# flkraus/bayesian-yolov3

Hardware: AMD Instinct MI355X
Metric: img/s at T=30 MC-dropout, 608x608 (higher is better)
Workload: dtype f32 via split-f16 (hi+lo fp16 pairs, 3 fp16 MFMA products, fp32 accumulate)

## Files before the change

### bayesian-yolov3_amd/byolo/_lib.py

```python
import ctypes
import os

_HERE = os.path.dirname(os.path.abspath(__file__))
LIB_PATH = os.environ.get("BYOLO_LIB") or os.path.join(_HERE, "libbyolo.so")

OK, ERR_ARG, ERR_STATE, ERR_HIP, ERR_NOMEM, ERR_RANGE = 0, -1, -2, -3, -4, -5
DET_STANDARD, DET_ALEATORIC, DET_EPISTEMIC = 0, 1, 2
NMS_AGNOSTIC, NMS_TWO_CLASS, NMS_PER_CLASS = 0, 1, 2
NMS_MAX_CLASSES = 128
NORM_BN, NORM_DROPOUT = 1, 2
AUG_SATURATION, AUG_BRIGHTNESS, AUG_HUE = 1, 2, 3
AUG_COLORED_SALT_N_PEPPER, AUG_SALT_N_PEPPER, AUG_GAUSSIAN = 1, 2, 3


class ByoloError(RuntimeError):
    def __init__(self, code, msg):
        super().__init__("libbyolo error %d: %s" % (code, msg))
        self.code = code


class Cfg(ctypes.Structure):
    _fields_ = [("img_h", ctypes.c_int32), ("img_w", ctypes.c_int32), ("img_c", ctypes.c_int32),
                ("cls_cnt", ctypes.c_int32), ("drop_prob", ctypes.c_float), ("max_out", ctypes.c_int32),
                ("iou_thresh", ctypes.c_float), ("nms_mode", ctypes.c_int32), ("keep_all_outputs", ctypes.c_int32)]


class PlanOpts(ctypes.Structure):
    _fields_ = [(n, ctypes.c_int32) for n in (
        "struct_bytes", "graphs", "serialize_convs", "serialize_heads", "dedup", "lowmain", "kx3", "p1", "b2b", "kx3_wide", "wino_split", "wino_split_min_c",
        "wino_split_bn", "wino_split_rounds", "winograd", "wino_fused", "stream1x1", "gemm_stream", "ksplit", "streamk",
        "plain_epilogue", "wshift_per_layer", "nms_general", "wino_split_persist", "wino_split_feed")] + [(n, ctypes.c_float) for n in (
        "wino_split_min_gflop", "wino_split_chunk_mb", "wino_min_gflop", "wino_chunk_mb", "wino_min_ratio")]


class AugPlan(ctypes.Structure):
    _fields_ = [(n, ctypes.c_int32) for n in ("y0", "x0", "ch", "cw", "row0", "rescale", "flip", "blur_k", "color_op", "noise_op")] + \
               [("color_param", ctypes.c_float), ("noise_param", ctypes.c_float), ("noise_key", ctypes.c_uint64)]


EVAL_MAX_GT, EVAL_MAX_UNC, EVAL_RECORD_HEAD = 1024, 16, 7


class EvalCfg(ctypes.Structure):
    _fields_ = [(n, ctypes.c_int32) for n in ("struct_bytes", "row_len", "obj_idx", "cls_start_idx", "cls_cnt", "n_unc")] + \
               [("unc_cols", ctypes.c_int32 * EVAL_MAX_UNC), ("iou_thresh", ctypes.c_float), ("min_score", ctypes.c_float)]


EVAL_LOC_WORDS, EVAL_LOC_MAX_LAYERS, EVAL_LOC_MAX_PRIORS = 6, 8, 16


class EvalLocCfg(ctypes.Structure):
    _fields_ = [(n, ctypes.c_int32) for n in ("struct_bytes", "layer_col", "prior_col", "n_layers")] + \
               [(n, ctypes.c_int32 * EVAL_LOC_MAX_LAYERS) for n in ("lh", "lw", "n_priors")] + \
               [(n, (ctypes.c_float * EVAL_LOC_MAX_PRIORS) * EVAL_LOC_MAX_LAYERS) for n in ("prior_w", "prior_h")]


EVAL_LADDER_MAX = 16


class EvalLadderCfg(ctypes.Structure):
    _fields_ = [("struct_bytes", ctypes.c_int32), ("n_thr", ctypes.c_int32), ("thresholds", ctypes.c_float * EVAL_LADDER_MAX)]


EVAL_SUBSETS_MAX = 16


class EvalSubsetsCfg(ctypes.Structure):
    _fields_ = [("struct_bytes", ctypes.c_int32), ("n_subsets", ctypes.c_int32), ("lo", ctypes.c_float * EVAL_SUBSETS_MAX),
                ("hi", ctypes.c_float * EVAL_SUBSETS_MAX), ("img_h", ctypes.c_float), ("ignore_thresh", ctypes.c_float),
                ("height_slack", ctypes.c_float), ("ignore_other_classes", ctypes.c_int32)]


class EvalSummary(ctypes.Structure):
    _fields_ = [(n, ctypes.c_int32) for n in ("struct_bytes", "overflow", "record_words", "reserved")] + \
               [(n, ctypes.c_int64) for n in ("n_records", "n_seen", "n_images")]


VOTE_NONE, VOTE_ALE, VOTE_EPI, VOTE_TOTAL = 0, 1, 2, 3


class VoteCfg(ctypes.Structure):
    _fields_ = [("struct_bytes", ctypes.c_int32), ("var", ctypes.c_int32)] + \
               [(n, ctypes.c_float) for n in ("sigma_t", "iou_min", "min_score", "var_floor")] + \
               [("ale_col", ctypes.c_int32), ("epi_col", ctypes.c_int32)]
# ... 192 lines not shown
```

### bayesian-yolov3_amd/csrc/byolo_api.hip

```cpp
#include "byolo_internal.h"
#include <cfloat>

static thread_local std::string g_err;

int32_t byolo_fail(byolo_t* h, int32_t code, const char* fmt, ...) {
    char buf[1024];
    va_list ap; va_start(ap, fmt); vsnprintf(buf, sizeof buf, fmt, ap); va_end(ap);
    if (h) h->err = buf; else g_err = buf;
    return code;
}

extern "C" const char* byolo_version(void) { return "byolo 0.7 (gfx950; fp32 MFMA and split-f16 MFMA; abi 7)"; }
extern "C" int32_t byolo_abi_version(void) { return BYOLO_ABI_VERSION; }

extern "C" const char* byolo_last_error(const byolo_t* h) { return h ? h->err.c_str() : g_err.c_str(); }

static void plan_opts_defaults(byolo_plan_opts& o);
static void plan_opts_from_env(byolo_plan_opts& o);

extern "C" int32_t byolo_create(const byolo_cfg* cfg, int32_t device, byolo_t** out) {
    if (!cfg || !out) return fail(nullptr, BYOLO_ERR_ARG, "byolo_create: null argument");
    if (cfg->img_h <= 0 || cfg->img_w <= 0 || cfg->img_c <= 0)
        return fail(nullptr, BYOLO_ERR_ARG, "byolo_create: invalid image size");
    if (cfg->img_h % 32 || cfg->img_w % 32)
        return fail(nullptr, BYOLO_ERR_ARG, "byolo_create: full_img_size must be a multiple of 32 (yolov3.py:207-208)");
    if (cfg->cls_cnt < 1 || cfg->cls_cnt > byk::BYOLO_MAX_CLASSES)
        return fail(nullptr, BYOLO_ERR_ARG, "byolo_create: cls_cnt outside 1 .. 128");
    if (cfg->max_out < 1 || cfg->max_out > 2048) return fail(nullptr, BYOLO_ERR_ARG, "byolo_create: max_out out of [1,2048]");
    if (!(cfg->drop_prob >= 0.f && cfg->drop_prob < 1.f)) return fail(nullptr, BYOLO_ERR_ARG, "byolo_create: drop_prob");
    byolo_t* h = new (std::nothrow) byolo();
    if (!h) return fail(nullptr, BYOLO_ERR_NOMEM, "byolo_create: out of host memory");
    h->cfg = *cfg;
    h->device = device;
    plan_opts_defaults(h->opts);
    plan_opts_from_env(h->opts);
    h->dedup = h->opts.dedup != 0;
    if (const char* e = getenv("BYOLO_PRECISION")) h->precision = (!strcmp(e, "f32") || !strcmp(e, "0")) ? 0 : 1;
    h->prec_requested = h->precision;
    *out = h;
    return BYOLO_OK;
}

static void plan_opts_defaults(byolo_plan_opts& o) {
    memset(&o, 0, sizeof o);
    o.struct_bytes = (int32_t)sizeof o;
    o.graphs = 1; o.serialize_convs = 1; o.serialize_heads = 1; o.dedup = 1; o.lowmain = 1; o.kx3 = 1; o.p1 = 1; o.b2b = 1; o.kx3_wide = 0;
    o.wino_split = 1; o.wino_split_min_c = 256; o.wino_split_bn = 0; o.wino_split_rounds = 0;
    o.winograd = 1; o.wino_fused = 1; o.stream1x1 = 1; o.gemm_stream = 1; o.ksplit = -1; o.streamk = 1; o.plain_epilogue = 1; o.wino_split_persist = 0; o.wino_split_feed = 3;
    o.wino_split_min_gflop = 30.f; o.wino_split_chunk_mb = 1500.f; o.wino_min_gflop = 10.f; o.wino_chunk_mb = 800.f; o.wino_min_ratio = 80.f;
}
static void plan_opts_from_env(byolo_plan_opts& o) {
    auto geti = [](const char* name, int32_t& v) { if (const char* e = getenv(name)) v = atoi(e); };
    auto getf = [](const char* name, float& v) { if (const char* e = getenv(name)) v = (float)atof(e); };
    geti("BYOLO_GRAPHS", o.graphs); geti("BYOLO_SERIALIZE_CONVS", o.serialize_convs); geti("BYOLO_SERIALIZE_HEADS", o.serialize_heads);
    if (const char* e = getenv("BYOLO_NO_DEDUP")) o.dedup = atoi(e) ? 0 : 1;
    geti("BYOLO_LOWMAIN", o.lowmain); geti("BYOLO_KX3", o.kx3); geti("BYOLO_P1", o.p1); geti("BYOLO_B2B", o.b2b); geti("BYOLO_KX3_WIDE", o.kx3_wide);
    geti("BYOLO_WINO_SPLIT", o.wino_split); geti("BYOLO_WINO_SPLIT_MIN_C", o.wino_split_min_c); geti("BYOLO_WINO_SPLIT_BN", o.wino_split_bn);
    geti("BYOLO_WINO_SPLIT_ROUNDS", o.wino_split_rounds); geti("BYOLO_WINOGRAD", o.winograd);
    geti("BYOLO_WINO_FUSED", o.wino_fused); geti("BYOLO_STREAM1X1", o.stream1x1); geti("BYOLO_GEMM_STREAM", o.gemm_stream);
    geti("BYOLO_KSPLIT", o.ksplit); geti("BYOLO_STREAMK", o.streamk); geti("BYOLO_PLAIN_EPILOGUE", o.plain_epilogue); geti("BYOLO_WINO_SPLIT_PERSIST", o.wino_split_persist); geti("BYOLO_WINO_SPLIT_FEED", o.wino_split_feed);
    geti("BYOLO_WSHIFT_PER_LAYER", o.wshift_per_layer); geti("BYOLO_NMS_GENERAL", o.nms_general);
    getf("BYOLO_WINO_SPLIT_MIN_GFLOP", o.wino_split_min_gflop); getf("BYOLO_WINO_SPLIT_CHUNK_MB", o.wino_split_chunk_mb);
    getf("BYOLO_WINO_MIN_GFLOP", o.wino_min_gflop); getf("BYOLO_WINO_CHUNK_MB", o.wino_chunk_mb); getf("BYOLO_WINO_MIN_RATIO", o.wino_min_ratio);
}

static void drop_graphs(byolo_t* h) {
    bool any = false;
    for (auto& g : h->graphs) any = any || g.exec;
    if (any) (void)hipDeviceSynchronize();
    for (auto& g : h->graphs) if (g.exec) (void)hipGraphExecDestroy(g.exec);
    h->graphs.clear();
}

extern "C" int32_t byolo_get_plan_opts(const byolo_t* h, byolo_plan_opts* out) {
    if (!h || !out) return fail(const_cast<byolo_t*>(h), BYOLO_ERR_ARG, "byolo_get_plan_opts: null argument");
    *out = h->opts;
    out->struct_bytes = (int32_t)sizeof *out;
    return BYOLO_OK;
}

extern "C" int32_t byolo_set_plan_opts(byolo_t* h, const byolo_plan_opts* o) {
    if (!h || !o) return fail(h, BYOLO_ERR_ARG, "byolo_set_plan_opts: null argument");
    if (o->struct_bytes != (int32_t)sizeof *o) return fail(h, BYOLO_ERR_ARG, "byolo_set_plan_opts: struct_bytes %d, this library's byolo_plan_opts has %d (include/byolo.h)", o->struct_bytes, (int)sizeof *o);
    if (o->graphs < 0 || o->graphs > 2 || o->serialize_convs < 0 || o->serialize_convs > 2 || o->b2b < 0 || o->b2b > 2 || o->kx3_wide < 0 || o->kx3_wide > 2 ||
        o->wino_split < 0 || o->wino_split > 2 || o->winograd < 0 || o->winograd > 2 || o->wino_fused < 0 || o->wino_fused > 2 || o->stream1x1 < 0 || o->stream1x1 > 2 ||
        o->streamk < 0 || o->streamk > 2 || o->ksplit < -1 || o->ksplit > 64 || (o->wino_split_bn != 0 && o->wino_split_bn != 128 && o->wino_split_bn != 256) ||
        o->wino_split_rounds < 0 || o->wino_split_persist < 0 || o->wino_split_persist > 2 || o->wino_split_feed < 0 || o->wino_split_feed > 3 || !(o->wino_split_chunk_mb > 0.f) || !(o->wino_chunk_mb > 0.f) || !(o->wino_split_min_gflop >= 0.f) || !(o->wino_min_gflop >= 0.f) || !(o->wino_min_ratio >= 0.f))
        return fail(h, BYOLO_ERR_ARG, "byolo_set_plan_opts: a field outside its range (include/byolo.h)");
    const byolo_plan_opts& c = h->opts;
    const bool repack = (o->wshift_per_layer != 0) != (c.wshift_per_layer != 0) || (o->dedup != 0) != (c.dedup != 0) || (o->lowmain != 0) != (c.lowmain != 0) || (o->kx3 != 0) != (c.kx3 != 0) || (o->p1 != 0) != (c.p1 != 0);
    h->opts = *o;
    h->dedup = o->dedup != 0;
    h->plan.B = -1; h->plan.T = -1; ++h->plan_epoch; h->wsm_B = -1;
    if (h->d_blob || !h->graphs.empty()) { HIPCHK(h, hipSetDevice(h->device)); drop_graphs(h); }
    if (repack && h->lowered) { h->lowered = false; h->finalized = false; }
    return BYOLO_OK;
}

extern "C" int32_t byolo_graph_stats(const byolo_t* h, int32_t* n_graphs, int64_t* replays, int64_t* captures, int64_t* updates) {
    if (!h) return BYOLO_ERR_ARG;
    int n = 0; for (const auto& g : h->graphs) n += g.exec != nullptr;
    if (n_graphs) *n_graphs = n;
    if (replays) *replays = h->graph_replays;
    if (captures) *captures = h->graph_captures;
    if (updates) *updates = h->graph_updates;
    return BYOLO_OK;
}

extern "C" int32_t byolo_set_precision(byolo_t* h, int32_t precision) {
    if (!h) return fail(nullptr, BYOLO_ERR_ARG, "byolo_set_precision: null handle");
    if (precision != BYOLO_PREC_F32 && precision != BYOLO_PREC_SPLIT_F16) return fail(h, BYOLO_ERR_ARG, "byolo_set_precision: unknown precision %d", precision);
    h->prec_requested = precision;
    if (precision == BYOLO_PREC_F32) h->prec_note.clear();
    if (precision != h->precision) { h->precision = precision; h->prec_note.clear(); h->finalized = false; h->plan.B = -1; h->plan.T = -1; ++h->plan_epoch; }
    return BYOLO_OK;
}
extern "C" int32_t byolo_get_precision(const byolo_t* h) { return h ? h->precision : BYOLO_ERR_ARG; }

extern "C" int32_t byolo_destroy(byolo_t* h) {
    if (!h) return BYOLO_OK;
    bool on_device = h->d_blob || h->d_ones || h->d_status || !h->graphs.empty() || h->cap_stream;
    for (auto& ps : h->prof) on_device = on_device || ps.ev[0] || !ps.step_ev.empty();
    if (on_device) {
        (void)hipSetDevice(h->device);
        drop_graphs(h);
        if (h->cap_stream) (void)hipStreamDestroy(h->cap_stream);
        if (h->d_blob) (void)hipFree(h->d_blob);
        if (h->d_ones) (void)hipFree(h->d_ones);
        if (h->d_zeros) (void)hipFree(h->d_zeros);
        if (h->ev_convs) (void)hipEventDestroy(h->ev_convs);
        if (h->d_status) (void)hipFree(h->d_status);
        if (h->pc_own) (void)hipFree(h->pc_own);
        if (h->vn_own) (void)hipFree(h->vn_own);
        if (h->vr_tab) (void)hipFree(h->vr_tab);
        if (h->sr_tab) (void)hipFree(h->sr_tab);
        if (h->sr_own) (void)hipFree(h->sr_own);
        if (h->h_status) (void)hipHostFree(h->h_status);
        for (auto& ps : h->prof) {
            for (auto& e : ps.ev) if (e) (void)hipEventDestroy(e);
            for (auto& e : ps.step_ev) (void)hipEventDestroy(e);
// ... 307 lines not shown
                h->aux.push_back({l.H, l.W, l.filters});
                st.raw_tensor = n + (int)h->aux.size() - 1;
                h->last_use.push_back(-1);
            } else if (st.in.n == 2 && any_tile && !all_tile) {
                const int kt = st.in.s[0].tile ? 0 : 1;
                Step part; part.layer = i; part.mode = STEP_PARTIAL;
                part.in.n = 1; part.in.s[0] = st.in.s[kt]; part.in.s[0].tile = false;
                part.c_lo = kt == 0 ? 0 : st.in.s[0].C; part.c_hi = part.c_lo + st.in.s[kt].C;
                h->aux.push_back({l.H, l.W, l.filters});
                part.out_tensor = n + (int)h->aux.size() - 1;
                h->last_use.push_back(-1);
                const int pidx = (int)h->steps.size();
                if (part.in.s[0].layer >= 0) h->last_use[part.in.s[0].layer] = pidx;
                h->steps.push_back(part);
                Step main = st; main.mode = STEP_MAIN; main.addend_tensor = part.out_tensor;
                main.in.n = 1; main.in.s[0] = st.in.s[1 - kt];
                main.c_lo = kt == 0 ? st.in.s[0].C : 0; main.c_hi = main.c_lo + st.in.s[1 - kt].C;
                st = main;
                if (h->opts.lowmain != 0 && l.ksize == 1 && l.stride == 1 && st.in.s[0].sh == 1 && st.in.s[0].layer >= 0 &&
                    !st.in.s[0].tile && (l.H & 1) == 0 && (l.W & 1) == 0 && (l.filters & 3) == 0 && l.fused_residual < 0 && (st.in.s[0].C % 32) == 0) {
                    Step lowst = st; lowst.mode = STEP_PARTIAL; lowst.low = true; lowst.addend_tensor = -1;
                    lowst.in.s[0].sh = 0;
                    h->aux.push_back({l.H / 2, l.W / 2, l.filters, true});
                    lowst.out_tensor = n + (int)h->aux.size() - 1;
                    h->last_use.push_back(-1);
                    const int lidx = (int)h->steps.size();
                    h->last_use[lowst.in.s[0].layer] = lidx;
                    h->steps.push_back(lowst);
                    Step fin; fin.layer = i; fin.mode = STEP_FINISH; fin.out_tensor = l.out_tensor;
                    fin.low_tensor = lowst.out_tensor; fin.addend_tensor = part.out_tensor;
                    fin.c_lo = st.c_lo; fin.c_hi = st.c_hi;
                    const int fidx = (int)h->steps.size();
                    h->last_use[fin.low_tensor] = fidx; h->last_use[fin.addend_tensor] = fidx;
                    h->steps.push_back(fin);
                    continue;
                }
            }
        }
        const int step_idx = (int)h->steps.size();
        for (int k = 0; k < st.in.n; ++k) if (st.in.s[k].layer >= 0) h->last_use[st.in.s[k].layer] = step_idx;
        if (st.addend_tensor >= 0) h->last_use[st.addend_tensor] = step_idx;
        if (l.fused_residual >= 0) h->last_use[h->layers[l.fused_residual].ref[0]] = step_idx;
        h->steps.push_back(st);
    }
    for (auto& st : h->steps) {
        if (!st.is_conv()) continue;
        const Layer& l = h->layers[st.layer];
        const int N = l.filters;
        if (l.direct) { st.tile = -1; st.Npad = N; }
        else { st.tile = conv_pick_tile(N); const int bn = conv_tile_bn(st.tile); st.Npad = (N + bn - 1) / bn * bn; }
        st.wino_ok = !l.direct && l.op == OP_CONV && l.ksize == 3 && l.stride == 1 && st.mode == STEP_NORMAL &&
                     st.in.n == 1 && st.in.s[0].sh == 0 && !st.in.s[0].tile && (l.Cin % 32) == 0 && (N % 4) == 0;
    }
    h->maxC = 1;
    for (const auto& l : h->layers) h->maxC = std::max(h->maxC, l.C);
    decide_loops(h);
    h->lowered = true;
    return BYOLO_OK;
}

int32_t byolo_lower(byolo_t* h) {
    const int n = (int)h->layers.size();
    if (!n) return fail(h, BYOLO_ERR_STATE, "byolo_finalize: empty graph");
    if (!h->n_det) return fail(h, BYOLO_ERR_STATE, "byolo_finalize: no detection layer (model.py:190: assert len(det_layers) > 0)");
    h->need_mat.assign(n, 0);
    for (int attempt = 0; ; ++attempt) {
        h->want_mat = -1;
        const int32_t rc = lower_once(h);
        if (rc == BYOLO_OK) return rc;
        if (h->want_mat < 0 || h->need_mat[h->want_mat] || attempt > n) return rc;
        h->need_mat[h->want_mat] = 1;
    }
}

static uint64_t sample_base(const byolo_t* h, int T, bool stacked) {
    if (h->tshard_T > 0 && stacked) return (uint64_t)h->first_image * (uint64_t)h->tshard_T + (uint64_t)h->tshard_t0;
    return (uint64_t)h->first_image * (uint64_t)T;
}

static EpiArgs raw_epi(const byolo_t* h, int layer) {
    EpiArgs e; memset(&e, 0, sizeof e);
    e.scale = h->d_ones; e.shift = h->d_zeros; e.flags = EPI_RAW;
    e.status = h->precision == 1 ? h->d_status : nullptr; e.layer_idx = layer;
    return e;
}

static void fill_conv(const byolo_t* h, const Step& st, const float* d_img, char* ws, int B, int T, ConvParams& p) {
    const Layer& l = h->layers[st.layer];
    memset(&p, 0, sizeof p);
    const float* srcs[2] = {nullptr, nullptr};
    int Cs[2] = {0, 0}, Hs[2] = {1, 1}, Wsz[2] = {1, 1}, sh[2] = {0, 0}, sdiv[2] = {1, 1};
    int64_t nsrc[2] = {0, 0};
    for (int k = 0; k < st.in.n; ++k) {
        const Src& s = st.in.s[k];
        if (s.layer < 0) { srcs[k] = (h->precision == 1 && !l.direct) ? reinterpret_cast<const float*>(ws + h->plan.img_split_off) : d_img; Hs[k] = h->cfg.img_h; Wsz[k] = h->cfg.img_w; nsrc[k] = B; }
        else {
            srcs[k] = reinterpret_cast<const float*>(ws + h->plan.off[s.layer]); Hs[k] = h->layers[s.layer].H; Wsz[k] = h->layers[s.layer].W;
            nsrc[k] = h->layers[s.layer].stacked ? (int64_t)B * T : B;
        }
        Cs[k] = s.C; sh[k] = s.sh; sdiv[k] = s.tile ? T : 1;
    }
    p.src0 = srcs[0]; p.src1 = srcs[1] ? srcs[1] : srcs[0];
    p.C0 = Cs[0]; p.C1 = Cs[1];
    p.Hs0 = Hs[0]; p.Ws0 = Wsz[0]; p.Hs1 = Hs[1]; p.Ws1 = Wsz[1];
    p.sh0 = sh[0]; p.sh1 = sh[1]; p.sdiv0 = sdiv[0]; p.sdiv1 = sdiv[1];
    p.Hin = Hs[0] << sh[0]; p.Win = Wsz[0] << sh[0];
// ... 94 lines not shown
            const int RT = w.P_pad / 128;
            f.slots = 512 / f.n_tiles; f.q = RT / f.slots; f.rem = RT % f.slots;
            f.xi_stride = (uint32_t)((uint64_t)w.P_pad * c.C0 * 4);
            f.d_ntiles = make_fastdiv((uint32_t)f.n_tiles); f.d_tt = w.d_tt; f.d_tw = w.d_tw;
            if (prof && (rc = mark_launch(h, s.layer, 130, rows, c.N, c.C0, algo_flops * ns / S, st))) return rc;
            HIPCHK(h, launch_wino_fused(f, st));
            continue;
        }
        if (h->opts.gemm_stream != 0 && gemm_stream_ok(c.C0, c.N)) {
            GemmStreamParams q; memset(&q, 0, sizeof q);
            q.a = V; q.a_bytes = (uint32_t)((uint64_t)rows * c.C0 * 4);
            q.w = dptr(h, s.wino_off); q.wstride = (uint32_t)((size_t)(c.C0 / 32) * c.N * 32 * 4); q.w_bytes = 16u * q.wstride;
            q.dst = Mb; q.C = c.C0; q.N = c.N; q.KT = c.C0 / 32; q.n_tiles = c.N / 128;
            q.RT = w.P_pad / 128;
            const int R = 16 * q.RT;
            q.slots = 512 / q.n_tiles; q.q = R / q.slots; q.rem = R % q.slots;
            q.d_ntiles = make_fastdiv((uint32_t)q.n_tiles); q.d_RT = make_fastdiv((uint32_t)q.RT);
            q.kind = 0; q.epi = raw_epi(h, s.layer); q.M = rows; q.Npad = c.N; q.ldc = c.N;
            if (prof && (rc = mark_launch(h, s.layer, 129, rows, c.N, c.C0, algo_flops * ns / S, st))) return rc;
            HIPCHK(h, launch_gemm_stream(q, st));
            if (prof && (rc = mark_launch(h, s.layer, -3, w.P, c.N, 0, 0.0, st))) return rc;
            HIPCHK(h, launch_wino_output(w, st));
            continue;
        }
        ConvParams g; memset(&g, 0, sizeof g);
        g.src0 = V; g.src1 = V; g.C0 = c.C0; g.C1 = 0;
        g.src0_bytes = g.src1_bytes = (uint32_t)((uint64_t)rows * c.C0 * 4);
        g.Hs0 = g.Hs1 = 1; g.Ws0 = g.Ws1 = rows; g.sdiv0 = g.sdiv1 = 1;
        g.Hin = 1; g.Win = rows; g.Hout = 1; g.Wout = rows; g.ksize = 1; g.stride = 1; g.pad = 0;
        g.M = rows; g.N = c.N; g.Npad = c.Npad; g.ldc = c.N; g.cin_tiles = c.C0 / 32; g.KT = g.cin_tiles;
        g.wpk = dptr(h, s.wino_off);
        g.wino_rows = (uint32_t)w.P_pad; g.d_wino = make_fastdiv((uint32_t)w.P_pad);
        g.wino_wstride = (uint32_t)((size_t)g.cin_tiles * c.Npad * 32 * 4);
        g.w_bytes = 16u * g.wino_wstride;
        g.epi = raw_epi(h, s.layer); g.rep = 1; g.addend_T = 1;
        g.dst = Mb;
        g.d_hw = make_fastdiv((uint32_t)rows); g.d_wout = make_fastdiv((uint32_t)rows);
        g.d_sdiv0 = g.d_sdiv1 = g.d_addT = make_fastdiv(1u);
        const ConvSplit sp = conv_plan_split(rows, c.Npad, g.KT, tile, 1.0, h->opts.ksplit, h->opts.streamk);
        if (conv_split_slab_bytes(sp, tile) <= h->plan.slab_bytes) {
            g.full_tiles = sp.full_tiles; g.split_tiles = sp.split_tiles; g.split_blocks = sp.split_blocks; g.ksplit = sp.ksplit;
            g.sk_grid = sp.sk_grid;
            g.slabs = c.slabs; g.slab_bytes = (uint32_t)conv_split_slab_bytes(sp, tile); g.counters = c.counters;
        }
        if (prof && (rc = mark_launch(h, s.layer, conv_tile_bn(tile), rows, c.N, c.C0, algo_flops * ns / S, st, g.sk_grid > 0 ? -g.sk_grid : (g.ksplit > 1 ? g.ksplit : 1), g.split_tiles))) return rc;
        HIPCHK(h, launch_conv_igemm(g, tile, st));
        if (prof && (rc = mark_launch(h, s.layer, -3, w.P, c.N, 0, 0.0, st))) return rc;
        HIPCHK(h, launch_wino_output(w, st));
    }
    return BYOLO_OK;
}

static int32_t run_wino_split(byolo_t* h, const Step& s, const Layer& l, const ConvParams& c, const WinoPlan& wp, double algo_flops,
                              char* ws, hipStream_t st, const WinoParams* feed = nullptr) {
    const bool prof = h->profiling >= 2;
    int32_t rc;
    const int S = c.M / (l.H * l.W), tt = wp.th * wp.tw;
    float* V = reinterpret_cast<float*>(ws + h->plan.wino_off);
    const bool drop = c.epi.flags & EPI_DROPOUT;
    for (int s0 = 0; s0 < S; s0 += wp.chunk) {
        const int ns = std::min(wp.chunk, S - s0);
        WinoParams w; memset(&w, 0, sizeof w);
        if (feed) w = *feed;
        w.x = feed ? nullptr : c.src0; w.v = V;
        w.H = l.H; w.W = l.W; w.C = c.C0; w.N = c.N; w.th = wp.th; w.tw = wp.tw;
        w.s0 = s0; w.P = ns * tt; w.P_pad = (int)align_up((size_t)w.P, 128);
        w.d_tt = make_fastdiv((uint32_t)tt); w.d_tw = make_fastdiv((uint32_t)wp.tw);
        w.d_c4 = make_fastdiv((uint32_t)(c.C0 / 4)); w.d_n4 = make_fastdiv((uint32_t)(c.N / 4));
        w.vmul = 1.f / ACT_SCALE;
        if (prof && (rc = mark_launch(h, s.layer, -4, w.P, c.C0, 0, 0.0, st))) return rc;
        HIPCHK(h, launch_wino_split_input(w, st));
        WinoSplitParams f; memset(&f, 0, sizeof f);
        const uint64_t rows = (uint64_t)16 * w.P_pad;
        f.v = V; f.v_bytes = (uint32_t)(rows * c.C0 * 4); f.xi_stride = (uint32_t)((uint64_t)w.P_pad * c.C0 * 4);
        f.w = dptr(h, s.wino_off); f.w_bytes = (uint32_t)((size_t)16 * c.C0 * c.N * 4);
        f.y = c.dst; f.residual = (c.epi.flags & EPI_RESIDUAL) ? c.residual : nullptr;
        f.epi = c.epi; f.epi.scale = dptr(h, drop ? l.wscalek_off : l.wscale_off);
        f.C = c.C0; f.N = c.N; f.KT = c.C0 / 32; f.n_tiles = c.N / wp.bn; f.bn = wp.bn;
        f.H = l.H; f.W = l.W; f.th = wp.th; f.tw = wp.tw; f.s0 = s0; f.P = w.P; f.P_pad = w.P_pad;
        f.bm = wp.bm; f.units = (w.P_pad / wp.bm) * f.n_tiles;
        const int chunk_idx = s0 / wp.chunk;
        f.persist = (h->opts.wino_split_persist == 2 && c.counters && chunk_idx < CNT_PER_STEP / 8) ? 2 : (h->opts.wino_split_persist ? 1 : 0);
        f.claims = c.counters ? c.counters + 8 * chunk_idx : nullptr;
        f.d_ntiles = make_fastdiv((uint32_t)f.n_tiles); f.d_tt = w.d_tt; f.d_tw = w.d_tw;
        if (prof && (rc = mark_launch(h, s.layer, 140, (int64_t)rows, c.N, c.C0, algo_flops * ns / S, st, 1, wp.bn))) return rc;
        HIPCHK(h, launch_wino_split(f, st));
    }
    return BYOLO_OK;
}

static int32_t run_decode(byolo_t* h, char* ws, float* boxes, int B, int T, hipStream_t st, int mode = 0) {
    for (const auto& l : h->layers) {
        if (l.op != OP_DETECTION) continue;
        DecodeParams d; memset(&d, 0, sizeof d);
        d.mode = mode;
        if (mode && l.det_kind != BYOLO_DET_EPISTEMIC) return fail(h, BYOLO_ERR_ARG, "T sharding (byolo_set_tshard) is defined for epistemic detection layers");
        d.raw = mode == 2 ? nullptr : reinterpret_cast<const float*>(ws + h->plan.off[l.out_tensor]);
        d.boxes = boxes; d.lh = l.H; d.lw = l.W; d.C = h->cfg.cls_cnt;
        d.n_total = h->n_boxes; d.box_base = l.box_base; d.layer_id = l.det_id; d.ld = layer_pitch(l);
        d.status = h->precision == 1 ? h->d_status : nullptr;
        for (int k = 0; k < 3; ++k) { d.ph[k] = l.priors[2 * k]; d.pw[k] = l.priors[2 * k + 1]; }
        if (l.det_kind == BYOLO_DET_EPISTEMIC) { d.B = B; d.T = l.stacked ? T : 1; }
        else { d.B = l.stacked ? B * T : B; d.T = 1; }
        if (l.det_kind != BYOLO_DET_EPISTEMIC && l.stacked && T > 1)
            return fail(h, BYOLO_ERR_ARG, "byolo_forward: non-epistemic decode of a stacked (T>1) detection layer");
        HIPCHK(h, launch_decode(l.det_kind, d, st));
    }
    return BYOLO_OK;
}

static int64_t mask_layout(const byolo_t* h, int B, int T, int ordinal, int64_t* elements) {
    int64_t off = 0;
    for (const auto& l : h->layers) {
        if (l.drop_ordinal < 0) continue;
        const int64_t n = (l.stacked ? (int64_t)B * T : B) * l.H * l.W * l.filters;
        if (l.drop_ordinal == ordinal) { if (elements) *elements = n; return off; }
        off += (n + 31) / 32 * 32;
    }
    if (elements) *elements = 0;
    return off;
}

extern "C" int32_t byolo_num_dropout(const byolo_t* h) { return h ? h->n_dropout : BYOLO_ERR_ARG; }

static int32_t mask_layout_impl(byolo_t* h, int32_t B, int32_t T, int32_t ordinal, int64_t* bit_offset, int64_t* elements) {
    if (!h) return fail(nullptr, BYOLO_ERR_ARG, "byolo_mask_layout: null handle");
    if (!h->lowered) { int32_t rc = lower(h); if (rc) return rc; }
    if (B < 1 || T < 1 || ordinal < 0 || ordinal > h->n_dropout) return fail(h, BYOLO_ERR_ARG, "byolo_mask_layout: bad argument");
    int64_t n = 0;
    const int64_t off = mask_layout(h, B, T, ordinal, &n);
    if (bit_offset) *bit_offset = off;
    if (elements) *elements = n;
    return BYOLO_OK;
}
extern "C" int32_t byolo_mask_layout(byolo_t* h, int32_t B, int32_t T, int32_t ordinal, int64_t* bit_offset, int64_t* elements) {
    return guarded(h, "byolo_mask_layout", [&] { return mask_layout_impl(h, B, T, ordinal, bit_offset, elements); });
// ... 333 lines not shown
        fill_finish(h, s, ws, B, T, h->precision == 1 ? 2 : 1, f);
        return layer_epi(h, s.layer, a, f.epi);
    };
    auto feed_params = [&](size_t pi, WinoParams& w) -> int32_t {
        const Step& ps = h->steps[pi];
        memset(&w, 0, sizeof w);
        w.feed = h->plan.feed[pi];
        if (w.feed == 1) {
            ConvParams c; int tile = 0; double algo = 0.0;
            int32_t rc = prep(pi, c, tile, algo); if (rc) return rc;
            w.src_low = reinterpret_cast<const float*>(ws + h->plan.off[ps.raw_tensor]); w.src_T = T; w.src = c.epi;
        } else {
            FinishParams f;
            int32_t rc = finish_params(ps, f); if (rc) return rc;
            w.src_low = f.low; w.src_part = f.part; w.src_T = f.T; w.src = f.epi;
        }
        return BYOLO_OK;
    };
    for (size_t si = 0; si < h->steps.size(); ++si) {
        const Step& s = h->steps[si];
        const Layer& l = h->layers[s.layer];
        if (h->stop_layer >= 0 && s.layer >= h->stop_layer) break;
        if (wait_pending && s.layer >= h->backbone_end) { HIPCHK(h, hipStreamWaitEvent(st, h->ev_convs, 0)); wait_pending = false; }
        if (h->profiling && !backbone_marked && h->backbone_end >= 0 && s.layer >= h->backbone_end) {
            HIPCHK(h, hipEventRecord(h->wslot().ev[1], st)); backbone_marked = true;
        }
        ConvParams p;
        if (h->plan.feed[si] == 2) continue;
        if (s.mode == STEP_FINISH) {
            FinishParams f;
            rc = finish_params(s, f); if (rc) return rc;
            if (per_step) { rc = mark_launch(h, s.layer, -5, (int64_t)f.S * f.H * f.W, f.N, 0, 0.0, st); if (rc) return rc; }
            HIPCHK(h, launch_finish_upsampled(f, st));
            continue;
        }
        if (!s.is_conv()) { fill_conv(h, s, d_img, ws, B, T, p); rc = run_aux_step(h, s, p, st); if (rc) return rc; continue; }
        int tile = 0; double algo = 0.0;
        rc = prep(si, p, tile, algo); if (rc) return rc;
        if (h->plan.feed[si] == 1) {
            p.epi = raw_epi(h, s.layer); p.rep = 1;
            p.dst = reinterpret_cast<float*>(ws + h->plan.off[s.raw_tensor]);
        }
        const ConvSplit& sp = h->plan.split[si];
        if (h->plan.fuse[si]) {
            ConvParams f; int ftile = 0; double falgo = 0.0;
            rc = prep(si + 1, f, ftile, falgo); if (rc) return rc;
            p.f_wpk = f.wpk; p.f_w_bytes = f.w_bytes; p.f_epi = f.epi; p.f_dst = f.dst;
            p.f_N = f.N; p.f_Npad = f.Npad; p.f_ldc = f.ldc;
            if (per_step) { rc = mark_launch(h, s.layer, 4256, p.M, l.filters, (int64_t)l.ksize * l.ksize * (s.c_hi - s.c_lo), algo + falgo, st, 1, 0); if (rc) return rc; }
            HIPCHK(h, launch_conv_igemm(p, tile, st));
            ++si;
            continue;
        }
        if (h->plan.wino[si].chunk > 0 && h->precision == 1) {
            WinoParams fw;
            const bool fed = h->plan.feed_src[si] >= 0;
            if (fed) { rc = feed_params((size_t)h->plan.feed_src[si], fw); if (rc) return rc; }
            rc = run_wino_split(h, s, l, p, h->plan.wino[si], algo, ws, st, fed ? &fw : nullptr); if (rc) return rc;
            continue;
        }
        if (h->plan.wino[si].chunk > 0) { rc = run_winograd(h, s, l, p, h->plan.wino[si], tile, algo, ws, st); if (rc) return rc; continue; }
        if (h->plan.stream1x1[si]) {
            const int bn = h->plan.stream1x1[si];
            GemmStreamParams q; memset(&q, 0, sizeof q);
            q.a = p.src0; q.a_bytes = p.src0_bytes;
            q.w = p.wpk; q.w_bytes = p.w_bytes; q.wstride = 0;
            q.dst = p.dst; q.C = p.C0; q.N = p.N; q.KT = p.KT; q.n_tiles = bn == 64 ? 1 : p.N / 128;
            const int R = (p.M + 127) / 128;
            q.RT = R + 1;
            q.slots = 512 / q.n_tiles; q.q = R / q.slots; q.rem = R % q.slots;
            q.d_ntiles = make_fastdiv((uint32_t)q.n_tiles); q.d_RT = make_fastdiv((uint32_t)q.RT);
            q.kind = l.op == OP_DETECTION ? 2 : 1; q.M = p.M; q.Npad = p.Npad; q.ldc = p.ldc;
            q.epi = p.epi; q.addend = p.addend; q.hw = l.H * l.W;
            q.d_hw = p.d_hw; q.d_addT = p.d_addT;
            if (per_step) { rc = mark_launch(h, s.layer, bn == 64 ? 132 : 131, p.M, l.filters, p.C0, algo, st); if (rc) return rc; }
            HIPCHK(h, launch_gemm_stream(q, st));
            continue;
        }
        if (per_step) { rc = mark_launch(h, s.layer, l.direct ? -1 : conv_tile_bn(tile) + (p.kx3 == 1 ? 3000 : (p.kx3 == 2 ? 2000 : (p.split ? 1000 : 0))), p.M, l.filters, (int64_t)l.ksize * l.ksize * (s.c_hi - s.c_lo), algo, st, l.direct ? 1 : (sp.sk_grid > 0 ? -sp.sk_grid : sp.ksplit), l.direct ? 0 : sp.split_tiles); if (rc) return rc; }
        HIPCHK(h, l.direct ? launch_conv_direct(p, st) : launch_conv_igemm(p, tile, st));
    }
    if (per_step) {
        byolo::ProfSlot& ps = h->wslot();
        int e; rc = next_event(h, st, &e); if (rc) return rc;
        if (ps.last_main >= 0) ps.launches[ps.last_main].ev_end = e;
        ps.step_valid = true;
    }
    if (h->profiling) { if (!backbone_marked) HIPCHK(h, hipEventRecord(h->wslot().ev[1], st)); HIPCHK(h, hipEventRecord(h->wslot().ev[2], st)); }
    if (!capturing) {
        if (!h->ev_convs) HIPCHK(h, hipEventCreateWithFlags(&h->ev_convs, hipEventDisableTiming));
        HIPCHK(h, hipEventRecord(h->ev_convs, st)); h->convs_stream = st; h->ev_convs_valid = true;
    }
    float* boxes = d_boxes ? d_boxes : reinterpret_cast<float*>(ws + h->plan.boxes_off);
    if (d_boxes || d_rows) { rc = run_decode(h, ws, boxes, B, T, st, h->tshard_T > 0 ? 1 : 0); if (rc) return rc; }
    if ((d_boxes || d_rows) && h->vr_on && h->tshard_T == 0) {
        VarRecalParams v;
        byolo_var_recal_from_handle(h, &v);
        v.in = boxes; v.out = boxes; v.n = (int64_t)B * h->n_boxes;
        HIPCHK(h, launch_var_recal(v, st));
    }
    if (h->profiling) HIPCHK(h, hipEventRecord(h->wslot().ev[3], st));
    if (d_rows) {
        NmsParams n; memset(&n, 0, sizeof n);
        n.boxes = boxes; n.B = B; n.N = h->n_boxes; n.D = h->row_len; n.obj_idx = h->obj_idx; n.cls_start = h->cls_start;
        n.C = nms_classes(h->cfg.nms_mode, h->cfg.cls_cnt); n.max_out = h->cfg.max_out; n.iou_thr = h->cfg.iou_thresh;
        n.ws = ws + h->plan.nms_off; n.ws_bytes = nms_workspace_bytes_ex(B, h->n_boxes, h->cfg.nms_mode, h->cfg.cls_cnt);
        n.rows = d_rows; n.kept = d_kept; n.count = d_count; n.general_only = h->opts.nms_general != 0;
        if (h->cfg.nms_mode == BYOLO_NMS_TWO_CLASS && h->cfg.cls_cnt != 2) return fail(h, BYOLO_ERR_ARG, "byolo_forward: 2-class NMS needs cls_cnt == 2");
        if (h->soft_on) {
            SoftNmsParams sp = soft_params(h->soft_cfg);
            sp.n = n; sp.n.ws = ws + h->plan.soft_off; sp.n.ws_bytes = soft_nms_workspace_bytes(B, h->n_boxes, n.C);
// ... 215 lines not shown
        if (p.lh[l] < 1 || p.lw[l] < 1) return fail(h, BYOLO_ERR_ARG, "byolo_encode_gt: empty detection layer %d", l);
        p.base[l] = (int)n;
        n += (int64_t)p.lh[l] * p.lw[l] * 3;
        for (int k = 0; k < 3; ++k) {
            p.ph[l][k] = priors_hw[(l * 3 + k) * 2]; p.pw[l][k] = priors_hw[(l * 3 + k) * 2 + 1];
            if (!(p.ph[l][k] >= 0 && p.ph[l][k] <= 1 && p.pw[l][k] >= 0 && p.pw[l][k] <= 1))
                return fail(h, BYOLO_ERR_ARG, "byolo_encode_gt: prior height and width must be numbers between 0 and 1");
        }
    }
    if (n > (int64_t)1 << 28) return fail(h, BYOLO_ERR_ARG, "byolo_encode_gt: too many prior boxes");
    p.boxes = d_boxes; p.labels = d_labels; p.counts = d_counts; p.B = B; p.max_boxes = max_boxes; p.n_layers = n_layers; p.N = (int)n;
    p.ign_thresh = ign_thresh; p.loc = d_loc; p.obj = d_obj; p.cls = d_cls; p.ign = d_ign; p.best = reinterpret_cast<unsigned*>(d_workspace);
    hipError_t e = launch_encode_gt(p, reinterpret_cast<hipStream_t>(stream));
    if (e != hipSuccess) return fail(h, BYOLO_ERR_HIP, "byolo_encode_gt: %s", hipGetErrorString(e));
    return BYOLO_OK;
}

extern "C" size_t byolo_encode_gt_workspace_bytes(int32_t B, int32_t max_boxes) { return encode_gt_workspace_bytes(B, max_boxes); }

extern "C" size_t byolo_loss_workspace_bytes(void) { return loss_workspace_bytes() + 64; }

extern "C" int32_t byolo_loss(byolo_t* h, int32_t kind, int32_t aleatoric_loss, int32_t cls_cnt, const float* d_raw, int32_t pitch,
                              int32_t S, int32_t lh, int32_t lw, const float* d_gt_loc, const float* d_gt_obj,
                              const int32_t* d_gt_cls, const float* d_gt_ign, int64_t gt_stride, double* d_loss,
                              float* d_grad, int32_t grad_pitch, void* d_workspace, size_t workspace_bytes, void* stream) {
    if (!d_raw || !d_gt_loc || !d_gt_obj || !d_gt_cls || !d_gt_ign || !d_loss || !d_workspace) return fail(h, BYOLO_ERR_ARG, "byolo_loss: null argument");
    if (kind != BYOLO_DET_STANDARD && kind != BYOLO_DET_ALEATORIC)
        return fail(h, BYOLO_ERR_ARG, "byolo_loss: the loss exists for the standard and the aleatoric raw outputs (an epistemic layer "
                                      "is an aleatoric one outside inference mode, lib_yolo/model.py:166-173)");
    if (aleatoric_loss && kind != BYOLO_DET_ALEATORIC) return fail(h, BYOLO_ERR_ARG, "byolo_loss: aleatoric_loss needs log_loc_var (aleatoric output)");
    if (S < 1 || lh < 1 || lw < 1 || cls_cnt < 1 || cls_cnt > BYOLO_MAX_CLASSES) return fail(h, BYOLO_ERR_ARG, "byolo_loss: bad shape");
    const int F = 3 * (kind == BYOLO_DET_ALEATORIC ? 10 + 2 * cls_cnt : 5 + cls_cnt);
    if (pitch == 0) pitch = F;
    if (grad_pitch == 0) grad_pitch = F;
    if (pitch < F || (d_grad && grad_pitch < F)) return fail(h, BYOLO_ERR_ARG, "byolo_loss: pitch below the %d values of a cell", F);
    if (gt_stride < (int64_t)lh * lw * 3) return fail(h, BYOLO_ERR_ARG, "byolo_loss: gt_stride below the layer's prior boxes");
    if ((reinterpret_cast<uintptr_t>(d_gt_loc) & 15) != 0) return fail(h, BYOLO_ERR_ARG, "byolo_loss: d_gt_loc must be 16-byte aligned");
    if (workspace_bytes < byolo_loss_workspace_bytes()) return fail(h, BYOLO_ERR_NOMEM, "byolo_loss: workspace too small");
    if (h) HIPCHK(h, hipSetDevice(h->device));
    LossParams p; memset(&p, 0, sizeof p);
    p.raw = d_raw; p.pitch = pitch; p.grad = d_grad; p.grad_pitch = grad_pitch; p.S = S; p.lh = lh; p.lw = lw; p.C = cls_cnt;
    p.aleatoric = kind == BYOLO_DET_ALEATORIC; p.aleatoric_loss = aleatoric_loss != 0;
    p.gt_loc = d_gt_loc; p.gt_obj = d_gt_obj; p.gt_cls = d_gt_cls; p.gt_ign = d_gt_ign; p.gt_stride = gt_stride;
    p.partial = reinterpret_cast<double*>(align_up(reinterpret_cast<uintptr_t>(d_workspace), 64)); p.out = d_loss;
    hipError_t e = launch_loss(p, reinterpret_cast<hipStream_t>(stream));
    if (e != hipSuccess) return fail(h, e == hipErrorInvalidValue ? BYOLO_ERR_ARG : BYOLO_ERR_HIP, "byolo_loss: %s", hipGetErrorString(e));
    return BYOLO_OK;
}

static int32_t calibrate_bn_impl(byolo_t* h, const float* d_img, int32_t B, void* d_workspace, size_t workspace_bytes,
                                      void* stream) {
    int32_t rc = check_run(h, B, 1, "byolo_calibrate_bn"); if (rc) return rc;
    if (!d_img || !d_workspace) return fail(h, BYOLO_ERR_ARG, "byolo_calibrate_bn: null argument");
    make_plan(h, B, 1);
    if (workspace_bytes < h->plan.total) return fail(h, BYOLO_ERR_NOMEM, "byolo_calibrate_bn: workspace %zu < %zu", workspace_bytes, h->plan.total);
    for (size_t si = 0; si < h->steps.size(); ++si) {
        const Step& s = h->steps[si];
        if (h->plan.feed[si] == 1) h->plan.off[s.out_tensor] = h->plan.off[s.raw_tensor];
        else if (h->plan.feed[si] == 2) h->plan.off[s.out_tensor] = h->plan.off[s.addend_tensor];
    }
    HIPCHK(h, hipSetDevice(h->device));
    h->last_ws = d_workspace;
    hipStream_t st = reinterpret_cast<hipStream_t>(stream);
    char* ws = reinterpret_cast<char*>(d_workspace);
    double* d_tmp = reinterpret_cast<double*>(ws + h->plan.stats_off);
    float* d_mean = reinterpret_cast<float*>(ws + h->plan.stats_off + (size_t)1024 * 2 * h->maxC * sizeof(double));
    float* d_var = d_mean + h->maxC;
    std::vector<float> sc, sf;
    const FwdArgs cal{d_img, B, 1, 0, 0, nullptr, d_workspace, nullptr, nullptr, nullptr, nullptr};
    auto range_check = [&](const char* what) -> int32_t {
        unsigned f = 0, ly = 0xFFFFFFFFu;
        int32_t rc = read_status(h, st, &f, &ly); if (rc) return rc;
        if (f) { (void)byolo_clear_status(h, stream); return range_error(h, what, f, ly); }
        return BYOLO_OK;
    };
    if (h->precision == 1) { rc = range_check("byolo_calibrate_bn: left by an earlier byolo_forward"); if (rc) return rc; }
    if (h->precision == 1 && h->img_split) {
        HIPCHK(h, launch_f32_to_split(d_img, reinterpret_cast<float*>(ws + h->plan.img_split_off), (int64_t)B * h->cfg.img_h * h->cfg.img_w * h->cfg.img_c, ACT_SCALE, st, h->d_status));
        rc = range_check("byolo_calibrate_bn"); if (rc) return rc;
    }
    for (const Step& s : h->steps) {
        Layer& l = h->layers[s.layer];
        const bool split = h->precision == 1;
        ConvParams p;
        if (s.mode == STEP_FINISH) {
            FinishParams f; fill_finish(h, s, ws, B, 1, 0, f);
            HIPCHK(h, launch_finish_upsampled(f, st));
            p.dst = f.dst; p.M = f.S * f.H * f.W;
        } else {
        fill_conv(h, s, d_img, ws, B, 1, p);
        if (!s.is_conv()) { int32_t rc = run_aux_step(h, s, p, st); if (rc) return rc; continue; }
        const int ctile = split ? conv_split_tile(s.tile, s.kx3 || s.p1) : s.tile;
        if (l.op == OP_DETECTION) { rc = layer_epi(h, s.layer, cal, p.epi); if (rc) return rc; if (split) p.epi.flags |= EPI_F32OUT; HIPCHK(h, l.direct ? launch_conv_direct(p, st) : launch_conv_igemm(p, ctile, st)); continue; }
        p.epi.flags = split ? (s.mode == STEP_PARTIAL ? EPI_RAW : EPI_F32OUT) : 0;
        if (split && l.direct) p.split &= 1;
        HIPCHK(h, l.direct ? launch_conv_direct(p, st) : launch_conv_igemm(p, ctile, st));
        if (s.mode == STEP_PARTIAL) continue;
        }
        const int N = l.filters;
        HIPCHK(h, launch_channel_stats(p.dst, p.M, N, d_mean, d_var, d_tmp, st));
        HIPCHK(h, hipMemcpyAsync(h->params[l.p_mean].data.data(), d_mean, sizeof(float) * N, hipMemcpyDeviceToHost, st));
        HIPCHK(h, hipMemcpyAsync(h->params[l.p_var].data.data(), d_var, sizeof(float) * N, hipMemcpyDeviceToHost, st));
        HIPCHK(h, hipStreamSynchronize(st));
        if (split) {
            for (int c = 0; c < N; ++c) { const float f = 1.f / acc_scale_of(l, c); h->params[l.p_mean].data[c] *= f; h->params[l.p_var].data[c] *= f * f; }
        }
        for (int c = 0; c < N; ++c)
            if (!std::isfinite(h->params[l.p_mean].data[c]) || !std::isfinite(h->params[l.p_var].data[c]))
                return fail(h, BYOLO_ERR_ARG, "byolo_calibrate_bn: the batch statistics of layer '%s', channel %d are not finite (inf / NaN "
                            "activations on the calibration frames)", l.scope.c_str(), c);
        fold_layer(h, l, sc, sf);
        if (split) fold_split(l, sc, sf);
        HIPCHK(h, hipMemcpyAsync(dptr(h, l.scale_off), sc.data(), sizeof(float) * N, hipMemcpyHostToDevice, st));
        HIPCHK(h, hipMemcpyAsync(dptr(h, l.shift_off), sf.data(), sizeof(float) * N, hipMemcpyHostToDevice, st));
        HIPCHK(h, hipStreamSynchronize(st));
        if (l.drop_ordinal >= 0) {
            std::vector<float> sk = sc; scale_keep(h, sk);
            HIPCHK(h, hipMemcpyAsync(dptr(h, l.scalek_off), sk.data(), sizeof(float) * N, hipMemcpyHostToDevice, st));
            HIPCHK(h, hipStreamSynchronize(st));
        }
        if (split && s.wino_ok && !l.wshift_u.empty()) {
            std::vector<float> wsc, wsk;
            wino_scales(h, l, wsc, wsk);
            HIPCHK(h, hipMemcpyAsync(dptr(h, l.wscale_off), wsc.data(), sizeof(float) * N, hipMemcpyHostToDevice, st));
            HIPCHK(h, hipMemcpyAsync(dptr(h, l.wscalek_off), wsk.data(), sizeof(float) * N, hipMemcpyHostToDevice, st));
            HIPCHK(h, hipStreamSynchronize(st));
        }
        const float* res = l.fused_residual >= 0
            ? reinterpret_cast<const float*>(ws + h->plan.off[h->layers[l.fused_residual].ref[0]]) : nullptr;
        HIPCHK(h, launch_bn_act_inplace(p.dst, p.M, N, dptr(h, l.scale_off), dptr(h, l.shift_off), res, 1, split, st, split ? h->d_status : nullptr, s.layer));
        if (split) { rc = range_check("byolo_calibrate_bn"); if (rc) return rc; }
    }
    if (h->precision == 1) return range_check("byolo_calibrate_bn");
    HIPCHK(h, hipStreamSynchronize(st));
    return BYOLO_OK;
}
extern "C" int32_t byolo_calibrate_bn(byolo_t* h, const float* d_img, int32_t B, void* d_workspace, size_t workspace_bytes,
                                      void* stream) {
    return guarded(h, "byolo_calibrate_bn", [&] {
        const int32_t rc = calibrate_bn_impl(h, d_img, B, d_workspace, workspace_bytes, stream);
        if (h) {
            bool doctored = rc != BYOLO_OK;
            for (char f : h->plan.feed) doctored = doctored || f != 0;
            if (doctored) h->plan.B = -1;
        }
        return rc;
    });
}

extern "C" int32_t byolo_set_profiling(byolo_t* h, int32_t on) {
    if (!h) return BYOLO_ERR_ARG;
    h->profiling = on < 0 ? 0 : (on > 2 ? 2 : on);
    for (auto& ps : h->prof) { ps.ev_valid = false; ps.step_valid = false; }
    h->prof_age = 0;
    return BYOLO_OK;
}

extern "C" int32_t byolo_resume_profiling(byolo_t* h, int32_t on) {
    if (!h) return BYOLO_ERR_ARG;
    h->profiling = on < 0 ? 0 : (on > 2 ? 2 : on);
    return BYOLO_OK;
}

extern "C" int32_t byolo_set_profile_depth(byolo_t* h, int32_t depth) {
    if (!h) return BYOLO_ERR_ARG;
    if (depth < 1 || depth > 4096) return fail(h, BYOLO_ERR_ARG, "byolo_set_profile_depth: depth out of [1, 4096]");
    if ((int)h->prof.size() > depth) {
        HIPCHK(h, hipSetDevice(h->device));
        for (size_t i = depth; i < h->prof.size(); ++i) {
            for (auto& e : h->prof[i].ev) if (e) (void)hipEventDestroy(e);
            for (auto& e : h->prof[i].step_ev) (void)hipEventDestroy(e);
        }
    }
    const size_t pool = h->wslot().step_ev.size();
    const bool staged = h->wslot().ev[0] != nullptr;
    if (pool || staged) HIPCHK(h, hipSetDevice(h->device));
    h->prof.resize((size_t)depth);
    for (auto& ps : h->prof) {
        ps.ev_valid = false; ps.step_valid = false;
        while (ps.step_ev.size() < pool) { hipEvent_t e; HIPCHK(h, hipEventCreate(&e)); ps.step_ev.push_back(e); }
        if (staged) for (auto& e : ps.ev) if (!e) HIPCHK(h, hipEventCreate(&e));
    }
    h->prof_w = 0; h->prof_age = 0;
    return BYOLO_OK;
}

extern "C" int32_t byolo_select_profile(byolo_t* h, int32_t age) {
    if (!h) return BYOLO_ERR_ARG;
    if (age < 0 || age >= (int)h->prof.size()) return fail(h, BYOLO_ERR_ARG, "byolo_select_profile: age outside the profile depth");
    h->prof_age = age;
    return BYOLO_OK;
}

extern "C" int32_t byolo_set_tshard(byolo_t* h, int32_t t0, int32_t T_total) {
    if (!h) return BYOLO_ERR_ARG;
    if (T_total < 0 || t0 < 0 || (T_total > 0 && t0 >= T_total)) return fail(h, BYOLO_ERR_ARG, "byolo_set_tshard: need 0 <= t0 < T_total (T_total = 0 switches it off)");
// ... 122 lines not shown
```

### bayesian-yolov3_amd/csrc/byolo_internal.h

```cpp
#pragma once
#include <hip/hip_runtime.h>

#include <algorithm>
#include <atomic>
#include <cmath>
#include <cstdarg>
#include <cstdio>
#include <cstring>
#include <map>
#include <string>
#include <thread>
#include <vector>

#include "../../include/byolo.h"
#include "byolo_kernels.h"
#include "byolo_rng.h"

using namespace byk;

namespace byi {


enum Op { OP_CONV, OP_RESIDUAL, OP_ROUTE, OP_UPSAMPLE, OP_STACK, OP_DETECTION };

struct Param {
    std::string name;
    std::vector<int64_t> shape;
    std::vector<float> data;
    int64_t count() const { int64_t c = 1; for (auto s : shape) c *= s; return c; }
};

struct Layer {
    Op op;
    std::string scope;
    int filters = 0, ksize = 0, stride = 1, norm = 0;
    int prev = -1;
    int ref[2] = {-1, -1};
    int nref = 0;
    int det_kind = 0, det_id = 0;
    float priors[6] = {0, 0, 0, 0, 0, 0};
    int C = 0, H = 0, W = 0;
    bool stacked = false;
    int p_kernel = -1, p_bias = -1, p_gamma = -1, p_beta = -1, p_mean = -1, p_var = -1;
    int drop_ordinal = -1;
    int Cin = 0;
    bool materialized = false;
    int out_tensor = -1;
    int fused_residual = -1;
    bool standalone = false;
    int add_a = -1;
    size_t w_off = 0, scale_off = 0, shift_off = 0;
    size_t scalek_off = 0;
    int tile = 0, Npad = 0;
    bool direct = false;
    std::vector<int> wshift;
    std::vector<int> wshift_u;
    size_t wscale_off = 0, wscalek_off = 0;
    float in_scale = 1.f;
    int64_t box_base = 0;
};

struct Src { int layer; int C; int sh; bool tile; };
struct View { Src s[2]; int n = 0; };

enum StepMode { STEP_NORMAL = 0, STEP_REP = 1, STEP_PARTIAL = 2, STEP_MAIN = 3, STEP_GATHER = 4, STEP_ADD = 5, STEP_FINISH = 6 };
struct Step {
    int layer; View in;
    int mode = STEP_NORMAL;
    bool is_conv() const { return mode <= STEP_MAIN; }
    int c_lo = 0, c_hi = 0;
    int out_tensor = -1;
    int addend_tensor = -1;
    bool low = false;
    int low_tensor = -1;
    int raw_tensor = -1;
    size_t w_off = 0; int Npad = 0, tile = 0;
    bool wino_ok = false;
    size_t wino_off = 0;
    bool p1 = false;
    bool kx3 = false;
};
struct WinoPlan { int chunk = 0; int th = 0, tw = 0; size_t v_bytes = 0, m_bytes = 0; bool fused = false; int bm = 0, bn = 0;  };
struct AuxTensor { int H, W, C; bool stacked = false; };

struct Plan {
    int B = -1, T = -1;
    std::vector<int64_t> off;
    size_t arena = 0, boxes_off = 0, nms_off = 0, stats_off = 0, total = 0;
    size_t soft_off = 0;
    size_t vote_n_off = 0, vote_off = 0;
    size_t score_off = 0;
    size_t img_split_off = 0;
    size_t slab_off = 0, slab_bytes = 0, cnt_off = 0, cnt_bytes = 0;
    std::vector<ConvSplit> split;
    std::vector<int> tile;
    std::vector<WinoPlan> wino;
    std::vector<int> stream1x1;
    std::vector<char> fuse;
    std::vector<char> feed;
    std::vector<int> feed_src;
    size_t wino_off = 0;
};
static constexpr int CNT_PER_STEP = 1024;
static constexpr float ACT_SCALE = 4.f;

static inline int nms_classes(int nms_mode, int cls_cnt) {
    return nms_mode == BYOLO_NMS_PER_CLASS ? cls_cnt : nms_mode == BYOLO_NMS_TWO_CLASS ? 2 : 1;
}
static inline size_t nms_workspace_bytes_ex(int B, int64_t N, int nms_mode, int cls_cnt) {
    return nms_workspace_bytes(B, N, nms_mode == BYOLO_NMS_PER_CLASS ? cls_cnt : 2);
}

}
using namespace byi;


struct byolo {
    byolo_cfg cfg;
    int device = 0;
    std::string err;
    std::vector<Layer> layers;
    std::vector<Param> params;
    std::map<std::string, int> pindex;
    int n_dropout = 0, n_det = 0;
    int backbone_end = -1;
    bool finalized = false;
    bool lowered = false;
    std::vector<char> need_mat;
    mutable int want_mat = -1;
    std::vector<Step> steps;
    std::vector<AuxTensor> aux;
    byolo_plan_opts opts;
    struct GraphKey {
        const void* d_img; const void* d_mask_bits; const void* d_workspace; const void* d_boxes; const void* d_rows; const void* d_kept; const void* d_count;
        int32_t B, T, dropout_on, precision, plan_epoch, tshard_t0, tshard_T;
        bool same(const GraphKey& o) const { return !memcmp(this, &o, sizeof *this); }
    };
    struct GraphEntry { GraphKey key; uint64_t seed; int64_t first_image; hipGraphExec_t exec = nullptr; uint64_t used = 0; int seen = 0; bool no_graph = false; };
    std::vector<GraphEntry> graphs;
    hipStream_t cap_stream = nullptr;
    uint64_t graph_clock = 0; int64_t graph_replays = 0, graph_captures = 0, graph_updates = 0;
    bool dedup = true;
    bool img_split = false;
    int precision = 1;
    int prec_requested = 1;
    std::string prec_note;
    unsigned* d_status = nullptr; unsigned* h_status = nullptr;
    bool async_status = false;
    bool plan_inject = false;
    int plan_epoch = 0;
    int wsm_B = -1, wsm_T = -1, wsm_epoch = -1; size_t wsm_total = 0;
    hipEvent_t ev_convs = nullptr; hipStream_t convs_stream = nullptr; bool ev_convs_valid = false;
    bool quiet_next = false;
// ... 14 lines not shown
    double sr_host[BYOLO_SCORE_RECAL_TABLE_BYTES / sizeof(double)] = {};
    const float* sr_ptr = nullptr; int32_t sr_B = 0, sr_cap = 0;
    float* sr_own = nullptr; size_t sr_own_cap = 0;
    const int32_t* vn_ptr = nullptr; int32_t vn_B = 0, vn_cap = 0;
    int32_t* vn_own = nullptr; size_t vn_own_cap = 0;
    int64_t first_image = 0;
    int stop_layer = -1;
    int tshard_t0 = 0, tshard_T = 0;
    int profiling = 0;
    struct Launch { int layer, variant; int64_t m, n, k; double algo_flops; int ksplit, split_tiles; int ev_begin, ev_end; };
    struct ProfSlot {
        hipEvent_t ev[5] = {nullptr, nullptr, nullptr, nullptr, nullptr};
        bool ev_valid = false;
        std::vector<Launch> launches;
        std::vector<hipEvent_t> step_ev;
        int n_ev = 0, last_main = -1;
        bool step_valid = false;
    };
    std::vector<ProfSlot> prof = std::vector<ProfSlot>(1);
    int prof_w = 0;
    int prof_age = 0;
    ProfSlot& wslot() { return prof[prof_w]; }
    ProfSlot& rslot() { const int d = (int)prof.size(); return prof[((prof_w - prof_age) % d + d) % d]; }
};


int32_t byolo_fail(byolo_t* h, int32_t code, const char* fmt, ...);
#define fail byolo_fail
#define HIPCHK(h, call) do { hipError_t e_ = (call); if (e_ != hipSuccess) \
    return fail(h, BYOLO_ERR_HIP, "%s failed: %s (%s:%d)", #call, hipGetErrorString(e_), __FILE__, __LINE__); } while (0)
static inline size_t align_up(size_t v, size_t a) { return (v + a - 1) / a * a; }
static inline float* dptr(const byolo_t* h, size_t off) { return h->d_blob + off; }

template <class F>
static int32_t guarded(byolo_t* h, const char* what, F&& f) {
    try { return f(); }
    catch (const std::bad_alloc&) { return fail(h, BYOLO_ERR_NOMEM, "%s: out of host memory", what); }
    catch (const std::exception& e) { return fail(h, BYOLO_ERR_ARG, "%s: %s", what, e.what()); }
    catch (...) { return fail(h, BYOLO_ERR_ARG, "%s: an exception that is not a std::exception", what); }
}


#define lower byolo_lower
int32_t byolo_lower(byolo_t* h);
void fold_layer(const byolo_t* h, const Layer& l, std::vector<float>& scale, std::vector<float>& shift);
float acc_scale_of(const Layer& l, int n);
void fold_split(const Layer& l, std::vector<float>& sc, std::vector<float>& sf);
void scale_keep(const byolo_t* h, std::vector<float>& sc);
void wino_scales(const byolo_t* h, const Layer& l, std::vector<float>& sc, std::vector<float>& sk);
int layer_pitch(const Layer& l);
int64_t tensor_bytes(const byolo_t* h, int id, int B, int T);
void step_geometry(const byolo_t* h, const Step& st, int B, int T, int* M, int* KT);
void decide_loops(byolo_t* h);
void make_plan(byolo_t* h, int B, int T, bool inject = false);
int64_t piece_cap(const byolo_t* h, int32_t T);
int32_t check_run(byolo_t* h, int32_t B, int32_t T, const char* what, bool need_device = true);
int32_t byolo_vote_from_handle(byolo_t* h, VoteParams* p, const char* what);
int32_t byolo_var_recal_upload(byolo_t* h, hipStream_t st);
void byolo_var_recal_from_handle(const byolo_t* h, VarRecalParams* p);
int32_t byolo_score_recal_upload(byolo_t* h, hipStream_t st);
void byolo_score_recal_from_handle(const byolo_t* h, ScoreRecalParams* p);
static inline int64_t nms_out_cap(const byolo_t* h) { return (int64_t)h->cfg.max_out * nms_classes(h->cfg.nms_mode, h->cfg.cls_cnt); }
int32_t byolo_run_backbone(byolo_t* h, const float* d_img, int32_t B, void* d_workspace, size_t workspace_bytes, hipStream_t st);
```

### bayesian-yolov3_amd/csrc/byolo_kernels.h

```cpp
#pragma once
#include <hip/hip_runtime.h>
#include <stdint.h>
#include <atomic>

namespace byk {

inline hipError_t set_dynamic_lds_once(const void* fn, size_t bytes, std::atomic<uint64_t>& done) {
    int dev = 0;
    hipError_t e = hipGetDevice(&dev);
    if (e != hipSuccess) return e;
    const uint64_t bit = 1ull << (dev & 63);
    if (done.load(std::memory_order_acquire) & bit) return hipSuccess;
    e = hipFuncSetAttribute(fn, hipFuncAttributeMaxDynamicSharedMemorySize, (int)bytes);
    if (e == hipSuccess) done.fetch_or(bit, std::memory_order_release);
    return e;
}


enum : int { EPI_LEAKY = 1, EPI_DROPOUT = 2, EPI_RESIDUAL = 4, EPI_RAW = 8 ,
              EPI_F32OUT = 16  };
struct EpiArgs {
    const float* scale; const float* shift;
    const uint32_t* mask_bits;
    unsigned* status;
// ... 33 lines not shown
    int sdiv0, sdiv1;
    int Hin, Win, Hout, Wout;
    int ksize, stride, pad;
    int M, N, Npad, ldc;
    int KT, cin_tiles;
    int split;
    int kx3;
    int plain;
    int no_plain;
    FastDiv d_hw, d_wout, d_sdiv0, d_sdiv1, d_addT;
    int full_tiles, split_tiles, split_blocks, ksplit;
    int sk_grid, sk_q, sk_r;
    FastDiv d_skq, d_skq1, d_kt;
    float* slabs;
    uint32_t slab_bytes;
    unsigned* counters;
    uint32_t wino_rows, wino_wstride;
    FastDiv d_wino;
    FastDiv d_ntiles, d_cin, d_ks, d_ksplit;
    const float* f_wpk; uint32_t f_w_bytes;
    EpiArgs f_epi;
    float* f_dst;
    int f_N, f_Npad, f_ldc;
};

struct WinoParams {
    const float* x; float* v;
    const float* m; float* y;
    const float* residual;
    EpiArgs epi;
    int H, W, C, N, th, tw;
    int s0;
    int P, P_pad;
    FastDiv d_tt, d_tw, d_c4, d_n4;
    float vmul;
    int feed, src_T;
    const float* src_low; const float* src_part;
    EpiArgs src;
};
struct WinoSplitParams {
    const float* v; uint32_t v_bytes;
    uint32_t xi_stride;
    const float* w; uint32_t w_bytes;
    float* y;
    const float* residual;
    EpiArgs epi;
    int C, N, KT, n_tiles;
    int H, W, th, tw, s0, P, P_pad;
    int bm, bn;
    int persist;
    unsigned* claims;
    int units;
    FastDiv d_ntiles, d_tt, d_tw;
};
bool wino_split_ok(int C, int N);
hipError_t launch_wino_split_input(const WinoParams& p, hipStream_t st);
hipError_t launch_wino_split(const WinoSplitParams& p, hipStream_t st);
struct GemmStreamParams {
    const float* a; uint32_t a_bytes;
    const float* w; uint32_t w_bytes;
    float* dst;
    int C, N, KT, n_tiles;
    int RT;
    int slots, q, rem;
    uint32_t wstride;
    FastDiv d_ntiles, d_RT;
    int kind, M, Npad, ldc;
    EpiArgs epi;
    const float* addend; int hw;
    FastDiv d_hw, d_addT;
};
int conv1x1_stream_tile(int M, int C, int N, bool force = false);
struct WinoFusedParams {
    const float* v; uint32_t v_bytes;
    const float* w; uint32_t w_bytes;
    float* y; const float* residual;
    EpiArgs epi;
    int C, N, KT, n_tiles;
    int H, W, th, tw, s0, P;
    int slots, q, rem;
    uint32_t xi_stride, wstride;
    FastDiv d_ntiles, d_tt, d_tw;
};
bool wino_fused_ok(int C, int N);
hipError_t launch_wino_fused(const WinoFusedParams& p, hipStream_t st);
bool gemm_stream_ok(int C, int N);
hipError_t launch_gemm_stream(const GemmStreamParams& p, hipStream_t st);
hipError_t launch_wino_input(const WinoParams& p, hipStream_t st);
hipError_t launch_side_delay(int microseconds, hipStream_t st);
hipError_t launch_wino_output(const WinoParams& p, hipStream_t st);
void wino_weight_transform(const float g[9], float u[16]);

struct ConvSplit { int full_tiles, split_tiles, split_blocks, ksplit; int sk_grid = 0; };
ConvSplit conv_plan_split(int M, int Npad, int KT, int tile, double tk_scale = 1.0, int ksplit_knob = -1, int streamk_knob = 1);
size_t conv_split_slab_bytes(const ConvSplit& sp, int tile);

enum : int { TILE_128x128 = 0, TILE_128x64 = 1, TILE_128x32 = 2, TILE_128x256 = 3 };
int conv_tile_bn(int tile);
int conv_pick_tile(int N);
int conv_split_tile(int tile, bool wide);
hipError_t launch_conv_igemm(const ConvParams& p, int tile, hipStream_t st);
hipError_t launch_view_gather(const ConvParams& p, hipStream_t st);
hipError_t launch_tensor_add(const float* a, const float* b, float* dst, int64_t n, bool split, hipStream_t st, unsigned* status = nullptr, int layer = 0);
hipError_t launch_zero_words(void* p, int64_t n_words, hipStream_t st);
hipError_t launch_u8_to_f32(const uint8_t* src, float* dst, int64_t n, hipStream_t st);
hipError_t launch_f32_to_split(const float* src, float* dst, int64_t n, float mul, hipStream_t st, unsigned* status = nullptr);
hipError_t launch_split_to_f32(const float* src, float* dst, int64_t n, float mul, hipStream_t st);
hipError_t launch_conv_direct(const ConvParams& p, hipStream_t st);
// ... 120 lines not shown
```

### bayesian-yolov3_amd/csrc/byolo_plan.hip

```cpp
#include "byolo_internal.h"

int layer_pitch(const Layer& l) { return (l.op == OP_DETECTION && !l.direct) ? (l.C + 3) / 4 * 4 : l.C; }

int64_t tensor_bytes(const byolo_t* h, int id, int B, int T) {
    const int n = (int)h->layers.size();
    if (id >= n) {
        const AuxTensor& a = h->aux[id - n];
        return (int64_t)align_up((size_t)((int64_t)B * (a.stacked ? T : 1) * a.H * a.W * a.C) * sizeof(float), 256);
    }
    const Layer& l = h->layers[id];
    const int64_t S = l.stacked ? (int64_t)B * T : B;
    return (int64_t)align_up((size_t)(S * l.H * l.W * layer_pitch(l)) * sizeof(float), 256);
}

void step_geometry(const byolo_t* h, const Step& st, int B, int T, int* M, int* KT) {
    const Layer& l = h->layers[st.layer];
    const bool per_image = st.mode == STEP_REP || (st.mode == STEP_PARTIAL && !st.low);
    const int64_t S = (l.stacked && !per_image) ? (int64_t)B * T : B;
    *M = (int)(S * (l.H >> (st.low ? 1 : 0)) * (l.W >> (st.low ? 1 : 0)));
    *KT = l.ksize * l.ksize * ((st.c_hi - st.c_lo) / 32);
}

void decide_loops(byolo_t* h) {
    const bool kx3_on = h->opts.kx3 != 0, p1_on = h->opts.p1 != 0;
    for (auto& st : h->steps) {
        st.kx3 = false; st.p1 = false;
        if (!st.is_conv()) continue;
        const Layer& l = h->layers[st.layer];
        if (l.direct || h->precision != 1) continue;
        st.kx3 = kx3_on && l.ksize == 3 && l.stride == 1 && st.in.n == 1 && st.in.s[0].sh == 0 && st.in.s[0].layer >= 0 && st.Npad >= 64 &&
                 (st.mode == STEP_NORMAL || st.mode == STEP_REP);
        st.p1 = p1_on && l.ksize == 1 && l.stride == 1 && st.in.n == 1 && st.in.s[0].layer >= 0 && st.Npad >= 64;
    }
}

void make_plan(byolo_t* h, int B, int T, bool inject) {
    Plan& p = h->plan;
    if (p.B == B && p.T == T && h->plan_inject == inject) return;
    h->plan_inject = inject;
    const int n = (int)h->layers.size() + (int)h->aux.size();
    p.B = B; p.T = T; p.off.assign(n, -1);
    struct Blk { int64_t off, size; };
    std::vector<Blk> free_list;
    int64_t end = 0;
    auto alloc = [&](int64_t sz) -> int64_t {
        for (size_t i = 0; i < free_list.size(); ++i) {
            if (free_list[i].size >= sz) {
                const int64_t o = free_list[i].off;
                free_list[i].off += sz; free_list[i].size -= sz;
                if (!free_list[i].size) free_list.erase(free_list.begin() + i);
                return o;
            }
        }
        if (!free_list.empty() && free_list.back().off + free_list.back().size == end) {
            const int64_t o = free_list.back().off; end = o + sz; free_list.pop_back(); return o;
        }
        const int64_t o = end; end += sz; return o;
    };
    auto release = [&](int64_t off, int64_t sz) {
        Blk b{off, sz};
        auto it = std::lower_bound(free_list.begin(), free_list.end(), b, [](const Blk& x, const Blk& y) { return x.off < y.off; });
        it = free_list.insert(it, b);
        if (it + 1 != free_list.end() && it->off + it->size == (it + 1)->off) { it->size += (it + 1)->size; free_list.erase(it + 1); }
        if (it != free_list.begin() && (it - 1)->off + (it - 1)->size == it->off) { (it - 1)->size += it->size; free_list.erase(it); }
    };
    p.fuse.assign(h->steps.size(), 0);
    { const int b2b = h->opts.b2b;
      for (size_t si = 0; b2b && h->precision == 1 && !inject && !h->cfg.keep_all_outputs && si + 1 < h->steps.size(); ++si) {
          const Step& s = h->steps[si];
          const Layer& l = h->layers[s.layer];
          if (!(s.is_conv() && s.kx3 && s.mode == STEP_NORMAL && l.op == OP_CONV && !l.direct && l.filters == 256 && s.Npad == 256 && l.fused_residual < 0)) continue;
          int M, KT; step_geometry(h, s, B, T, &M, &KT);
          if (b2b < 2 && (int64_t)((M + 127) / 128) < 4 * 256) continue;
          const Step& s2 = h->steps[si + 1];
          const Layer& l2 = h->layers[s2.layer];
          const int out_t = s.out_tensor;
          if (s2.is_conv() && s2.mode == STEP_NORMAL && s2.p1 && !l2.direct && l2.ksize == 1 && l2.stride == 1 && s2.in.n == 1 &&
              s2.in.s[0].layer == out_t && !s2.in.s[0].tile && s2.in.s[0].sh == 0 && s2.in.s[0].C == 256 && s2.c_lo == 0 && s2.c_hi == 256 &&
              l2.fused_residual < 0 && s2.Npad <= 128 && (layer_pitch(l2) % 4) == 0 && l2.H == l.H && l2.W == l.W && l2.stacked == l.stacked &&
              h->last_use[out_t] == (int)si + 1)
              p.fuse[si] = 1;
      }
    }
    p.wino.assign(h->steps.size(), WinoPlan{});
    size_t wino_scratch = 0;
    if (h->precision == 1) {
// ... 3 lines not shown
        const int bn_pref = h->opts.wino_split_bn;
        auto model_ms = [](int64_t row_tiles, int N, int C, int bn) -> double {
            if (bn == 256) return (double)((row_tiles * (N / 256) + 255) / 256) * (0.030 + 0.000293 * C);
            const int64_t units = row_tiles * (N / 128), full = units / 512, rem = units % 512;
            const double t = (double)full * (0.012 + 0.000367 * C) + (rem == 0 ? 0.0 : rem <= 256 ? 0.024 + 0.00022 * C : 0.012 + 0.000367 * C);
            return units > 1024 ? 1.09 * t : t;
        };
        for (size_t si = 0; on && si < h->steps.size(); ++si) {
            const Step& s = h->steps[si];
            const Layer& l = h->layers[s.layer];
            if (!s.wino_ok || !s.kx3 || s.mode != STEP_NORMAL || !wino_split_ok(s.c_hi - s.c_lo, l.filters) || s.Npad != l.filters || (l.fused_residual >= 0 && l.drop_ordinal >= 0) || p.fuse[si]) continue;
            int M, KT; step_geometry(h, s, B, T, &M, &KT);
            const double flops = 2.0 * M * l.filters * 9.0 * l.Cin;
            if (flops < min_flops) continue;
            if (on < 2 && l.Cin < h->opts.wino_split_min_c) continue;
            const int th = (l.H + 1) / 2, tw = (l.W + 1) / 2, S = M / (l.H * l.W);
            const double per_sample = 16.0 * th * tw * l.Cin * 4.0;
            const int nchunks = std::max(1, (int)std::ceil(S * per_sample / budget));
            const int chunk = (S + nchunks - 1) / nchunks;
            const int64_t row_tiles = (int64_t)align_up((size_t)chunk * th * tw, 128) / bm;
            const bool can256 = (l.filters % 256) == 0;
            int bn = (bn_pref == 256 && can256) ? 256 : bn_pref == 128 ? 128 : 0;
            if (bn_pref == 256 && !can256) bn = 128;
            const double t256 = can256 ? model_ms(row_tiles, l.filters, l.Cin, 256) : 1e30, t128 = model_ms(row_tiles, l.filters, l.Cin, 128);
            if (bn == 0) bn = t256 <= t128 ? 256 : 128;
            if (on < 2) {
                const double t_res = l.fused_residual >= 0 ? 4.0 * M * l.filters / 2.5e9 : 0.0;
                const double t_wino = nchunks * ((bn == 256 ? t256 : t128) + 0.012 + (double)row_tiles * bm * per_sample / ((double)th * tw) / 4.5e9) + t_res;
                const double t_direct = 0.028 + flops / ((l.Cin >= 512 ? 390.0 : 425.0) * 1e9);
                if (t_wino > 0.97 * t_direct) continue;
            }
            WinoPlan& w = p.wino[si];
            w.th = th; w.tw = tw; w.bm = bm; w.fused = true;
            w.bn = bn;
            w.chunk = chunk;
            const int rounds = h->opts.wino_split_rounds;
            if (rounds > 0) {
                const int slots = (w.bn == 256 ? 256 : 512), n_tiles = l.filters / w.bn;
                const int64_t row_tiles = (int64_t)rounds * slots / n_tiles;
                const int tt = w.th * w.tw;
                int c = (int)((row_tiles * w.bm) / tt);
                while (c > 1 && (int64_t)align_up((size_t)c * tt, 128) / w.bm * n_tiles > (int64_t)rounds * slots) --c;
                w.chunk = std::max(1, std::min(S, c));
            }
            const size_t P_pad = align_up((size_t)w.chunk * w.th * w.tw, 128);
            w.v_bytes = align_up((size_t)16 * P_pad * l.Cin * 4, 256);
            if (w.v_bytes > CONV_MAX_SRC_BYTES) { w = WinoPlan{}; continue; }
            w.m_bytes = 0;
            wino_scratch = std::max(wino_scratch, w.v_bytes);
        }
    }
    p.feed.assign(h->steps.size(), 0); p.feed_src.assign(h->steps.size(), -1);
    std::vector<int> last_use = h->last_use;
    if (h->precision == 1 && h->opts.wino_split_feed && !h->cfg.keep_all_outputs) {
        std::vector<int> readers(n, 0);
        for (const Step& s : h->steps) {
            for (int k = 0; k < s.in.n; ++k) if (s.in.s[k].layer >= 0) ++readers[s.in.s[k].layer];
            if (s.addend_tensor >= 0) ++readers[s.addend_tensor];
            if (s.low_tensor >= 0) ++readers[s.low_tensor];
            const Layer& l = h->layers[s.layer];
            if (s.is_conv() && l.fused_residual >= 0) ++readers[h->layers[l.fused_residual].ref[0]];
        }
        for (int si = 0; si < (int)h->steps.size(); ++si) {
            const Step& s = h->steps[si];
            const int kind = s.mode == STEP_REP ? 1 : s.mode == STEP_FINISH ? 2 : 0;
            if (!kind || !(h->opts.wino_split_feed & kind) || (kind == 1 && s.raw_tensor < 0) || (kind == 2 && (s.low_tensor < 0 || s.addend_tensor < 0))) continue;
            const Layer& l = h->layers[s.layer];
            const int t = s.out_tensor, ri = h->last_use[t];
            if (t >= (int)h->layers.size() || l.op != OP_CONV || l.direct || l.fused_residual >= 0 || (l.filters & 3) || readers[t] != 1 || ri <= si) continue;
            const Step& r = h->steps[ri];
            if (p.wino[ri].chunk <= 0 || !r.wino_ok || r.in.n != 1 || r.in.s[0].layer != t || r.in.s[0].sh != 0 || r.in.s[0].tile) continue;
            p.feed[si] = (char)kind; p.feed_src[ri] = si;
            if (kind == 1) last_use[s.raw_tensor] = ri;
            else { last_use[s.low_tensor] = ri; if (s.addend_tensor >= 0) last_use[s.addend_tensor] = ri; }
        }
    }
    for (int si = 0; si < (int)h->steps.size(); ++si) {
        const Layer& l = h->layers[h->steps[si].layer];
        const int t = p.feed[si] == 1 ? h->steps[si].raw_tensor : h->steps[si].out_tensor;
        if (!(si > 0 && p.fuse[si - 1]) && p.feed[si] != 2) p.off[t] = alloc(tensor_bytes(h, t, B, T));
        if (p.fuse[si]) { const int t2 = h->steps[si + 1].out_tensor; p.off[t2] = alloc(tensor_bytes(h, t2, B, T)); }
        if (h->cfg.keep_all_outputs) continue;
        for (int k = 0; k < n; ++k)
            if (p.off[k] >= 0 && last_use[k] == si) release(p.off[k], tensor_bytes(h, k, B, T));
        if (last_use[t] < 0 && l.op != OP_DETECTION && p.feed[si] != 2) release(p.off[t], tensor_bytes(h, t, B, T));
    }
    p.arena = align_up((size_t)end, 256);
    p.boxes_off = p.arena;
    size_t o = p.boxes_off + align_up((size_t)B * h->n_boxes * h->row_len * sizeof(float), 256);
    p.nms_off = o; o += align_up(nms_workspace_bytes_ex(B, h->n_boxes, h->cfg.nms_mode, h->cfg.cls_cnt), 256);
    p.soft_off = o;
    if (h->soft_on) o += align_up(soft_nms_workspace_bytes(B, h->n_boxes, nms_classes(h->cfg.nms_mode, h->cfg.cls_cnt)), 256);
    p.vote_n_off = p.vote_off = o;
    if (h->vote_on) {
        o += align_up((size_t)B * nms_out_cap(h) * sizeof(int32_t), 256);
        p.vote_off = o; o += align_up(box_vote_workspace_bytes(B, h->n_boxes), 256);
    }
    p.score_off = o;
    if (h->sr_on) o += align_up((size_t)B * nms_out_cap(h) * sizeof(float), 256);
    p.stats_off = o; o += align_up((size_t)1024 * 2 * h->maxC * sizeof(double) + 2 * h->maxC * sizeof(float), 256);
    p.img_split_off = o; if (h->img_split) o += align_up((size_t)B * h->cfg.img_h * h->cfg.img_w * h->cfg.img_c * sizeof(float), 256);
    p.split.assign(h->steps.size(), ConvSplit{0, 0, 0, 1});
    p.tile.assign(h->steps.size(), 0);
    size_t slab = 0;
    for (size_t si = 0; si < h->steps.size(); ++si) {
        const Step& s = h->steps[si];
        const Layer& l = h->layers[s.layer];
        if (!s.is_conv() || l.direct) continue;
        int M, KT; step_geometry(h, s, B, T, &M, &KT);
        int tile = s.tile;
        if (tile == TILE_128x128 && (l.filters % 128) == 0 && (int64_t)((M + 127) / 128) * (l.filters / 128) < 512) tile = TILE_128x64;
        if (h->precision == 1) tile = conv_split_tile(tile, s.kx3 || s.p1);
        else if (inject && tile == TILE_128x128) tile = TILE_128x64;
        const int kx3_wide = h->opts.kx3_wide;
        if (h->precision == 1 && s.kx3 && (s.Npad % 256) == 0 && kx3_wide && (l.filters % 128) == 0 &&
            (kx3_wide >= 2 ? (tile == TILE_128x128 || tile == TILE_128x64)
                           : (tile == TILE_128x128 && (int64_t)((M + 127) / 128) * (s.Npad / 256) >= 4 * 256)))
            tile = TILE_128x256;
        if (p.fuse[si]) tile = TILE_128x256;
        p.tile[si] = tile;
        const bool sp = h->precision == 1, kx3 = sp && s.kx3;
        p.split[si] = conv_plan_split(M, s.Npad, kx3 ? KT / 3 : KT, tile, sp ? (kx3 ? 1.2 : 0.4) : 1.0, h->opts.ksplit, h->opts.streamk);
        if (s.low) p.split[si] = ConvSplit{((M + 127) / 128) * (s.Npad / conv_tile_bn(tile)), 0, 0, 1};
        if (tile == TILE_128x256) p.split[si] = ConvSplit{((M + 127) / 128) * (s.Npad / 256), 0, 0, 1};
        slab = std::max(slab, conv_split_slab_bytes(p.split[si], tile));
    }
    { const int on = (h->precision == 1 || inject) ? 0 : h->opts.winograd;
      const double min_flops = on >= 2 ? 0.0 : (double)h->opts.wino_min_gflop * 1e9, budget = (double)h->opts.wino_chunk_mb * 1e6;
      for (size_t si = 0; on && si < h->steps.size(); ++si) {
        const Step& s = h->steps[si];
        const Layer& l = h->layers[s.layer];
        if (!s.wino_ok) continue;
// ... 61 lines not shown
    return BYOLO_OK;
}

int64_t piece_cap(const byolo_t* h, int32_t T) {
    uint64_t per_image = (uint64_t)h->cfg.img_h * h->cfg.img_w * h->cfg.img_c * 4;
    int64_t rows = 0;
    for (const auto& l : h->layers) {
        const uint64_t s = l.stacked ? (uint64_t)T : 1;
        if (l.materialized) per_image = std::max(per_image, s * l.H * l.W * l.C * 4);
        rows = std::max<int64_t>(rows, (int64_t)s * l.H * l.W);
    }
    const uint64_t by_bytes = CONV_MAX_SRC_BYTES / per_image, by_rows = (((uint64_t)1 << 31) - 1) / (uint64_t)rows;
    return (int64_t)std::min<uint64_t>(std::min(by_bytes, by_rows), 1 << 20);
}

int32_t check_run(byolo_t* h, int32_t B, int32_t T, const char* what, bool need_device) {
    if (!h) return fail(nullptr, BYOLO_ERR_ARG, "%s: null handle", what);
    if (need_device && !h->finalized) return fail(h, BYOLO_ERR_STATE, "%s: call byolo_finalize first", what);
    if (!h->lowered) { int32_t rc = lower(h); if (rc) return rc; }
    if (B < 1 || T < 1) return fail(h, BYOLO_ERR_ARG, "%s: B and T must be >= 1", what);
    for (const auto& l : h->layers) {
        const int64_t S = l.stacked ? (int64_t)B * T : B;
        if (S * l.H * l.W >= (int64_t)1 << 31) return fail(h, BYOLO_ERR_ARG, "%s: B*T*h*w exceeds 2^31 pixels", what);
        if (l.materialized && (uint64_t)S * l.H * l.W * l.C * 4 > CONV_MAX_SRC_BYTES)
            return fail(h, BYOLO_ERR_ARG, "%s: a [%lld,%d,%d,%d] activation exceeds the 3 GiB a convolution source may span; "
                        "split the call into smaller image batches", what, (long long)S, l.H, l.W, l.C);
    }
    if ((uint64_t)B * h->cfg.img_h * h->cfg.img_w * h->cfg.img_c * 4 > CONV_MAX_SRC_BYTES)
        return fail(h, BYOLO_ERR_ARG, "%s: the image batch exceeds 3 GiB; split the call", what);
    return BYOLO_OK;
}

static int32_t workspace_bytes_impl(byolo_t* h, int32_t B, int32_t T, size_t* out) {
    if (h && B >= 1 && T >= 1) {
        if (!h->lowered) { int32_t rc = lower(h); if (rc) return rc; }
        const int64_t cap = piece_cap(h, T);
        if (cap >= 1 && B > cap) {
            if (!out) return fail(h, BYOLO_ERR_ARG, "byolo_workspace_bytes: null out");
            size_t a = 0, b = 0;
            int32_t rc = byolo_workspace_bytes(h, (int32_t)cap, T, &a); if (rc) return rc;
            if (B % cap) { rc = byolo_workspace_bytes(h, (int32_t)(B % cap), T, &b); if (rc) return rc; }
            *out = std::max(a, b);
            return BYOLO_OK;
        }
    }
    int32_t rc = check_run(h, B, T, "byolo_workspace_bytes", false); if (rc) return rc;
    if (!out) return fail(h, BYOLO_ERR_ARG, "byolo_workspace_bytes: null out");
    make_plan(h, B, T, false);
    if (h->wsm_B != B || h->wsm_T != T || h->wsm_epoch != h->plan_epoch) {
        const Plan keep = h->plan;
        h->plan.B = -1;
        make_plan(h, B, T, true);
        h->wsm_total = h->plan.total; h->wsm_B = B; h->wsm_T = T; h->wsm_epoch = h->plan_epoch;
        h->plan = keep; h->plan_inject = false;
    }
    *out = std::max(h->plan.total, h->wsm_total);
    return BYOLO_OK;
}
extern "C" int32_t byolo_workspace_bytes(byolo_t* h, int32_t B, int32_t T, size_t* out) {
    return guarded(h, "byolo_workspace_bytes", [&] { return workspace_bytes_impl(h, B, T, out); });
}


extern "C" int32_t byolo_plan_num(byolo_t* h, int32_t B, int32_t T, int32_t inject, int32_t* n_steps, int32_t* n_tensors, int64_t* arena_bytes) {
    return guarded(h, "byolo_plan_num", [&]() -> int32_t {
        int32_t rc = check_run(h, B, T, "byolo_plan_num", false); if (rc) return rc;
        h->plan.B = -1;
        make_plan(h, B, T, inject != 0);
        if (n_steps) *n_steps = (int32_t)h->steps.size();
        if (n_tensors) *n_tensors = (int32_t)(h->layers.size() + h->aux.size());
        if (arena_bytes) *arena_bytes = (int64_t)h->plan.arena;
        return BYOLO_OK;
    });
}
extern "C" int32_t byolo_plan_step(byolo_t* h, int32_t step, int32_t* out_tensor, int32_t* fuses_next, int32_t reads[8], int32_t* n_reads) {
    if (!h || h->plan.B < 0 || step < 0 || step >= (int32_t)h->steps.size()) return fail(h, BYOLO_ERR_ARG, "byolo_plan_step: no plan (byolo_plan_num first) or bad step");
    const Step& st = h->steps[step];
    const Layer& l = h->layers[st.layer];
    int n = 0;
    const int fs = step < (int32_t)h->plan.feed_src.size() ? h->plan.feed_src[step] : -1;
    const int fk = step < (int32_t)h->plan.feed.size() ? h->plan.feed[step] : 0;
    if (fs >= 0) {
        const Step& ps = h->steps[fs];
        if (h->plan.feed[fs] == 1) reads[n++] = ps.raw_tensor;
        else { reads[n++] = ps.low_tensor; if (ps.addend_tensor >= 0) reads[n++] = ps.addend_tensor; }
    } else
    for (int k = 0; k < st.in.n; ++k) if (st.in.s[k].layer >= 0) reads[n++] = st.in.s[k].layer;
    if (st.addend_tensor >= 0) reads[n++] = st.addend_tensor;
    if (st.low_tensor >= 0) reads[n++] = st.low_tensor;
    if (st.is_conv() && st.mode != STEP_PARTIAL && l.fused_residual >= 0) reads[n++] = h->layers[l.fused_residual].ref[0];
    if (out_tensor) *out_tensor = fk == 1 ? st.raw_tensor : fk == 2 ? st.low_tensor : st.out_tensor;
    if (fuses_next) *fuses_next = (step < (int32_t)h->plan.fuse.size() && h->plan.fuse[step]) ? 1 : 0;
    if (n_reads) *n_reads = n;
    return BYOLO_OK;
}
extern "C" int32_t byolo_plan_tensor(byolo_t* h, int32_t tensor, int64_t* offset, int64_t* bytes, int32_t* read_after_the_steps) {
    const int32_t nt = h ? (int32_t)(h->layers.size() + h->aux.size()) : 0;
    if (!h || h->plan.B < 0 || tensor < 0 || tensor >= nt) return fail(h, BYOLO_ERR_ARG, "byolo_plan_tensor: no plan (byolo_plan_num first) or bad tensor");
    if (offset) *offset = h->plan.off[tensor];
    if (bytes) *bytes = tensor_bytes(h, tensor, h->plan.B, h->plan.T);
    if (read_after_the_steps) *read_after_the_steps = (tensor < (int32_t)h->layers.size() && (h->layers[tensor].op == OP_DETECTION || h->cfg.keep_all_outputs)) ? 1 : 0;
    return BYOLO_OK;
}
```

### bayesian-yolov3_amd/csrc/conv_igemm.hip

```cpp
#include <hip/hip_runtime.h>
#include <algorithm>
#include <cmath>
#include <type_traits>
#include "byolo_kernels.h"
#include "byolo_rng.h"
#include "mfma_pipe.h"
#include "epilogue.h"

namespace byk {

using namespace pipe;

#ifndef BYOLO_CONV_ABLATE
#define BYOLO_CONV_ABLATE 0
#endif
static constexpr int ABL = BYOLO_CONV_ABLATE;

__device__ __forceinline__ int xcd_remap(int bid, int nwg) {
    const int q = nwg >> 3, r = nwg & 7, xcd = bid & 7, i = bid >> 3;
    return (xcd < r ? xcd * (q + 1) : r * (q + 1) + (xcd - r) * q) + i;
}

struct TileShare { int counter, my_slab, nseg, base, stride, first_add; };

// ... 473 lines not shown
    constexpr int BM = 128, ROWB = LD * 4, A_BUF = BM * ROWB, BN2 = 32 * WN2;
    using BT2 = SplitTile<BM, BN2, WM2, WN2>;
    constexpr int TM2 = BT2::TM;
    static_assert(BT2::TN == 1 && WM2 * WN2 == 8, "8 waves, one column block each");
    char* lds = reinterpret_cast<char*>(smem);
    int tid = threadIdx.x;
    asm volatile("" : "+v"(tid));
    const int wave = tid >> 6, lane = tid & 63, li = lane & 31, lh = lane >> 5;
    auto to_lds = [&](auto drop_tag) {
        constexpr bool DROP = decltype(drop_tag)::value;
        const float slope = (p.epi.flags & EPI_LEAKY) ? 0.1f : 1.f;
        const int nb = wave * 32 + 4 * lh;
        float vmax = 0.f;
        f32x4 sc4[4], sf4[4];
#pragma unroll
        for (int g = 0; g < 4; ++g) {
            sc4[g] = *reinterpret_cast<const f32x4*>(p.epi.scale + nb + 8 * g);
            sf4[g] = *reinterpret_cast<const f32x4*>(p.epi.shift + nb + 8 * g);
        }
#pragma unroll
        for (int i = 0; i < 4; ++i) {
            const uint32_t rr = (uint32_t)(i * 32 + li), m = tile_m * BM + rr;
            const uint64_t idx_row = p.epi.idx_base + (uint64_t)m * (uint64_t)p.N + (uint64_t)nb;
            const epi::DropRow drow(idx_row, p.epi.k1);
#pragma unroll
            for (int g = 0; g < 4; ++g) {
                const int dn = 8 * g;
                f32x4 a4;
#pragma unroll
                for (int q = 0; q < 4; ++q) a4[q] = acc[i][0][4 * g + q];
                bool keep[4] = {true, true, true, true};
                if constexpr (DROP) epi::keep4(drow, dn, p.epi.k0, p.epi.thr, keep);
                const f32x4 v = epi::bn_act4_pk(a4, sc4[g], sf4[g], keep, slope);
                vmax = epi::absmax4(vmax, v);
                const f32x4 e = epi::split_encode4(v);
                char* at = lds + wave * A_BUF + rr * ROWB + (lh + 2 * g) * 8;
                typedef float f32x2 __attribute__((ext_vector_type(2)));
                *reinterpret_cast<f32x2*>(at) = f32x2{e[0], e[1]};
                *reinterpret_cast<f32x2*>(at + 64) = f32x2{e[2], e[3]};
            }
        }
        if (p.epi.status && vmax >= 65520.f) { atomicOr(p.epi.status, 1u); atomicMin(p.epi.status + 1, (unsigned)p.epi.layer_idx); }
    };
    if (p.epi.flags & EPI_DROPOUT) to_lds(std::true_type{}); else to_lds(std::false_type{});
    __syncthreads();
    const BT2 bt(smem, tid);
    f32x16 acc2[TM2][1];
#pragma unroll
    for (int i = 0; i < TM2; ++i)
#pragma unroll
        for (int r = 0; r < 16; ++r) acc2[i][0][r] = 0.f;
    const __amdgpu_buffer_rsrc_t w_rsrc = make_rsrc(p.f_wpk, p.f_w_bytes);
    const uint32_t w_step = (uint32_t)p.f_Npad * BK * 4;
    f16x8 bfr[2][2][1][2];
    f16x8 afr[2][TM2][2];
    bt.load_b(bfr[0], w_rsrc, 0u);
    bt.template read_frags<0, 0>(afr[0]);
    auto step2 = [&](auto s_tag) {
        constexpr int S = decltype(s_tag)::value, KT2 = S >> 1, H = S & 1;
        __builtin_amdgcn_sched_barrier(0);
        if constexpr (H == 0 && KT2 < 7) bt.load_b(bfr[(KT2 + 1) & 1], w_rsrc, (uint32_t)(KT2 + 1) * w_step);
        if constexpr (S < 15) bt.template read_frags<((S + 1) >> 1) & 7, (S + 1) & 1>(afr[(S + 1) & 1]);
        __builtin_amdgcn_sched_barrier(0);
        mfma_step_split<TM2, 1>(acc2, afr[S & 1], bfr[KT2 & 1][H]);
        __builtin_amdgcn_sched_barrier(0);
    };
    step2(std::integral_constant<int, 0>{}); step2(std::integral_constant<int, 1>{}); step2(std::integral_constant<int, 2>{});
    step2(std::integral_constant<int, 3>{}); step2(std::integral_constant<int, 4>{}); step2(std::integral_constant<int, 5>{});
    step2(std::integral_constant<int, 6>{}); step2(std::integral_constant<int, 7>{}); step2(std::integral_constant<int, 8>{});
    step2(std::integral_constant<int, 9>{}); step2(std::integral_constant<int, 10>{}); step2(std::integral_constant<int, 11>{});
    step2(std::integral_constant<int, 12>{}); step2(std::integral_constant<int, 13>{}); step2(std::integral_constant<int, 14>{});
    step2(std::integral_constant<int, 15>{});
    __syncthreads();
    auto follower = [&](auto drop_tag, auto split_tag) {
        constexpr bool DROP = decltype(drop_tag)::value, SPLIT_OUT = decltype(split_tag)::value;
        const float slope = (p.f_epi.flags & EPI_LEAKY) ? 0.1f : 1.f;
        const int nb = bt.wn * 32 + 4 * lh;
        float vmax = 0.f;
#pragma unroll
        for (int i = 0; i < TM2; ++i) {
            const uint32_t m = tile_m * BM + (uint32_t)((bt.wm * TM2 + i) * 32 + li);
            if (m >= (uint32_t)p.M) continue;
            const uint64_t idx_row = p.f_epi.idx_base + (uint64_t)m * (uint64_t)p.f_N + (uint64_t)nb;
            const epi::DropRow drow(idx_row, p.f_epi.k1);
            float* d = p.f_dst + (size_t)m * p.f_ldc + nb;
#pragma unroll
            for (int g = 0; g < 4; ++g) {
                const int dn = 8 * g, n0 = nb + dn;
                if (n0 >= p.f_N) continue;
                const f32x4 sc4 = *reinterpret_cast<const f32x4*>(p.f_epi.scale + n0);
                const f32x4 sf4 = *reinterpret_cast<const f32x4*>(p.f_epi.shift + n0);
                f32x4 a4;
#pragma unroll
                for (int q = 0; q < 4; ++q) a4[q] = acc2[i][0][4 * g + q];
                bool keep[4] = {true, true, true, true};
                if constexpr (DROP) epi::keep4(drow, dn, p.f_epi.k0, p.f_epi.thr, keep);
                const f32x4 v = epi::bn_act4_pk(a4, sc4, sf4, keep, slope);
                if constexpr (SPLIT_OUT) vmax = epi::absmax4(vmax, v);
                if constexpr (SPLIT_OUT) *reinterpret_cast<f32x4*>(d + dn) = epi::split_encode4(v);
                else *reinterpret_cast<f32x4*>(d + dn) = v;
            }
        }
        if (SPLIT_OUT && p.epi.status && vmax >= 65520.f) { atomicOr(p.epi.status, 1u); atomicMin(p.epi.status + 1, (unsigned)p.f_epi.layer_idx); }
    };
    if (p.f_epi.flags & EPI_F32OUT) {
        if (p.f_epi.flags & EPI_DROPOUT) follower(std::true_type{}, std::false_type{}); else follower(std::false_type{}, std::false_type{});
    } else if (p.f_epi.flags & EPI_DROPOUT) follower(std::true_type{}, std::true_type{});
    else follower(std::false_type{}, std::true_type{});
}

template <int BM, int BN, int WM, int WN, bool WALK = false>
__device__ __forceinline__ void conv_tile_kx3(const ConvParams& p, float* smem, const int logical_or_first, const int sg_begin,
                                              const int sg_end, const TileShare sh) {
    using BT = SplitTileKx<BM, BN, WM, WN>;
    constexpr int NT = BT::NT, TM = BT::TM, TN = BT::TN, A_LD = BT::A_LD, A_LDX = BT::A_LDX, ROWB = BT::ROWB;
    const BT bt(smem);
    const uint32_t n_tiles = (uint32_t)p.Npad / BN;
    const uint32_t hw = (uint32_t)(p.Hout * p.Wout), W = (uint32_t)p.Wout;
    int v = logical_or_first;
    uint32_t tile_m, tile_n;
    auto locate = [&](int logical) { tile_m = fdiv((uint32_t)logical, p.d_ntiles); tile_n = (uint32_t)logical - tile_m * n_tiles; };
    locate(WALK ? xcd_remap(v, p.full_tiles) : logical_or_first);

    uint32_t a_off0[A_LDX], a_vm[A_LDX], a_voff[A_LDX];
    uint32_t fa[3][TM];
// ... 382 lines not shown
```

### bayesian-yolov3_amd/csrc/conv_kernels.hip

```cpp
#include <hip/hip_runtime.h>
#include "byolo_kernels.h"
#include "byolo_rng.h"
#include "epilogue.h"

namespace byk {
#ifndef BYOLO_NT_MISC
#define BYOLO_NT_MISC 1
#endif
__device__ __forceinline__ void st4(float* at, const epi::f32x4 v) {
    if constexpr (BYOLO_NT_MISC != 0) __builtin_nontemporal_store(v, reinterpret_cast<epi::f32x4*>(at));
    else *reinterpret_cast<epi::f32x4*>(at) = v;
}


typedef float f32x4 __attribute__((ext_vector_type(4)));

__device__ __forceinline__ uint32_t fdiv(uint32_t n, FastDiv d) { return (__umulhi(n, d.mul) + n) >> d.shr; }

template <int NOUT>
__global__ __launch_bounds__(256) void conv_stem3x3_kernel(const ConvParams p) {
    constexpr int ROWB = NOUT * 4 + 16, PIECES = NOUT / 4;
    __shared__ __attribute__((aligned(16))) char lds[256 * ROWB];
    const uint32_t m0 = blockIdx.x * 256u, m = m0 + threadIdx.x;
    const bool live = m < (uint32_t)p.M;
// ... 336 lines not shown
    scale[c] = inv;
    shift[c] = b[c] - m[c] * inv;
}
hipError_t launch_fold_bn(const float* gamma, const float* beta, const float* mean, const float* var, float eps,
                          float* scale, float* shift, int C, hipStream_t st) {
    hipLaunchKernelGGL(fold_bn_kernel, dim3((C + 255) / 256), dim3(256), 0, st, gamma, beta, mean, var, eps, scale,
                       shift, C);
    return hipGetLastError();
}

__global__ void bn_act_inplace_kernel(float* x, int64_t total, int C, const float* scale, const float* shift,
                                      const float* residual, int leaky) {
    for (int64_t i = (int64_t)blockIdx.x * blockDim.x + threadIdx.x; i < total; i += (int64_t)gridDim.x * blockDim.x) {
        const int c = (int)(i % C);
        float v = x[i] * scale[c] + shift[c];
        if (leaky) v = fmaxf(v, 0.1f * v);
        if (residual) v += residual[i];
        x[i] = v;
    }
}
__global__ void bn_act_inplace_split_kernel(f32x4* x, int64_t total4, int C4, const float* scale, const float* shift,
                                            const f32x4* residual, int leaky, unsigned* status, int layer) {
    float vmax = 0.f;
    for (int64_t i = (int64_t)blockIdx.x * blockDim.x + threadIdx.x; i < total4; i += (int64_t)gridDim.x * blockDim.x) {
        const int c = (int)(i % C4) * 4;
        f32x4 v = x[i];
#pragma unroll
        for (int q = 0; q < 4; ++q) {
            v[q] = v[q] * scale[c + q] + shift[c + q];
            if (leaky) v[q] = fmaxf(v[q], 0.1f * v[q]);
        }
        if (residual) v += epi::split_decode4(residual[i]);
        vmax = epi::absmax4(vmax, v);
        x[i] = epi::split_encode4(v);
    }
    if (status && vmax >= 65520.f) { atomicOr(status, 1u); atomicMin(status + 1, (unsigned)layer); }
}
hipError_t launch_bn_act_inplace(float* x, int64_t M, int C, const float* scale, const float* shift,
                                 const float* residual, int leaky, bool split, hipStream_t st, unsigned* status, int layer) {
    const int64_t total = M * C;
    int64_t blocks = (total + 255) / 256;
    if (blocks > 8192) blocks = 8192;
    if (split) {
        if (C & 3) return hipErrorInvalidValue;
        hipLaunchKernelGGL(bn_act_inplace_split_kernel, dim3((unsigned)blocks), dim3(256), 0, st, reinterpret_cast<f32x4*>(x), total / 4,
                           C / 4, scale, shift, reinterpret_cast<const f32x4*>(residual), leaky, status, layer);
        return hipGetLastError();
    }
    hipLaunchKernelGGL(bn_act_inplace_kernel, dim3((unsigned)blocks), dim3(256), 0, st, x, total, C, scale, shift,
                       residual, leaky);
    return hipGetLastError();
}

}
```

### bayesian-yolov3_amd/csrc/mfma_pipe.h

```cpp
#pragma once
#include <hip/hip_runtime.h>
#include <stdint.h>
#include "byolo_kernels.h"

namespace byk {
namespace pipe {

typedef float f32x4 __attribute__((ext_vector_type(4)));
typedef float f32x16 __attribute__((ext_vector_type(16)));
typedef unsigned u32x4 __attribute__((ext_vector_type(4)));

static constexpr int BK = 32;
static constexpr int LD = 36;
static constexpr int RSRC_FLAGS = 0x00020000;

__device__ __forceinline__ uint32_t fdiv(uint32_t n, FastDiv d) { return (__umulhi(n, d.mul) + n) >> d.shr; }

__device__ __forceinline__ __amdgpu_buffer_rsrc_t make_rsrc(const void* base, uint32_t bytes) {
    return __builtin_amdgcn_make_buffer_rsrc(const_cast<void*>(base), 0, bytes, RSRC_FLAGS);
}
template <int AUX = 0>
__device__ __forceinline__ f32x4 buffer_load_x4(__amdgpu_buffer_rsrc_t r, uint32_t voff, uint32_t soff) {
    return __builtin_bit_cast(f32x4, __builtin_amdgcn_raw_buffer_load_b128(r, voff, soff, AUX));
}

template <int N_MFMA, int N_VMEM, int N_DSR, int N_DSW>
__device__ __forceinline__ void sched_interleave() {
    constexpr int AUX = N_VMEM + N_DSR + N_DSW;
    constexpr int PER = (AUX + N_MFMA - 1) / N_MFMA;
#pragma unroll
    for (int k = 0; k < N_MFMA; ++k) {
        __builtin_amdgcn_sched_group_barrier(0x008, 1, 0);
#pragma unroll
        for (int u = 0; u < PER; ++u) {
            const int q = k * PER + u;
            if (q < N_VMEM) __builtin_amdgcn_sched_group_barrier(0x020, 1, 0);
            else if (q < N_VMEM + N_DSR) __builtin_amdgcn_sched_group_barrier(0x100, 1, 0);
            else if (q < AUX) __builtin_amdgcn_sched_group_barrier(0x200, 1, 0);
        }
    }
}

template <int BM_, int BN_, int WM_, int WN_>
struct BlockTile {
    static constexpr int BM = BM_, BN = BN_, WM = WM_, WN = WN_;
    static constexpr int NT = 64 * WM * WN;
    static constexpr int TM = BM / WM / 32, TN = BN / WN / 32;
    static constexpr int A_LD = BM * 8 / NT, B_LD = BN * 8 / NT;
    static constexpr int ROWB = LD * 4, A_BUF = BM * ROWB, B_BUF = BN * ROWB, B_BASE = 2 * A_BUF;
    static constexpr int JSTEP = (NT / 8) * ROWB;
    static constexpr int LDS_BYTES = 2 * (BM + BN) * ROWB;
    static constexpr int G = 4 * TM * TN;
    static constexpr int NFR = TM + TN;
    static constexpr int NLD = A_LD + B_LD;
    static_assert(TM >= 1 && TN >= 1 && A_LD >= 1 && B_LD >= 1 && BM * 8 % NT == 0 && BN * 8 % NT == 0, "tile config");
// ... 123 lines not shown
    }
    template <int BUF, int S> __device__ __forceinline__ void read_frags(f16x8 (&af)[TM][2]) const {
#pragma unroll
        for (int i = 0; i < TM; ++i)
#pragma unroll
            for (int h = 0; h < 2; ++h)
                af[i][h] = *reinterpret_cast<const f16x8*>(lds + fa_off + (BUF * A_BUF + S * 32 + h * 64 + i * 32 * ROWB));
    }
    __device__ __forceinline__ void load_b(f16x8 (&bf)[2][TN][2], __amdgpu_buffer_rsrc_t rsrc, uint32_t soff) const {
#pragma unroll
        for (int s = 0; s < 2; ++s)
#pragma unroll
            for (int j = 0; j < TN; ++j)
#pragma unroll
                for (int h = 0; h < 2; ++h)
                    bf[s][j][h] = __builtin_bit_cast(f16x8, __builtin_amdgcn_raw_buffer_load_b128(rsrc, b_voff, soff + (uint32_t)(j * SPLIT_WBLOCK + (s * 2 + h) * 1024), 0));
    }
};

template <int TM, int TN, bool FIRST = false>
__device__ __forceinline__ void mfma_step_split(f32x16 (&acc)[TM][TN], const f16x8 (&af)[TM][2], const f16x8 (&bf)[TN][2]) {
    const f32x16 zero = {0.f, 0.f, 0.f, 0.f, 0.f, 0.f, 0.f, 0.f, 0.f, 0.f, 0.f, 0.f, 0.f, 0.f, 0.f, 0.f};
#pragma unroll
    for (int pr = 0; pr < 3; ++pr)
#pragma unroll
        for (int i = 0; i < TM; ++i)
#pragma unroll
            for (int j = 0; j < TN; ++j)
                acc[i][j] = __builtin_amdgcn_mfma_f32_32x32x16_f16(bf[j][pr == 2 ? 1 : 0], af[i][pr == 1 ? 1 : 0], (FIRST && pr == 0) ? zero : acc[i][j], 0, 0, 0);
}

template <int BUF, bool HN, int N_LDB, int N_LDA, int N_ST, int ABL = 0, bool FIRST = false, class BT, class LB, class LA, class St>
__device__ __forceinline__ void tile_body_split(const BT& t, f32x16 (&acc)[BT::TM][BT::TN], f16x8 (&af0)[BT::TM][2], f16x8 (&af1)[BT::TM][2],
                                                const f16x8 (&bcur)[2][BT::TN][2], LB&& loads_b, LA&& loads_a, St&& store_next) {
    constexpr int G = BT::G;
    constexpr bool FR = !(ABL & 8);
    constexpr int NFR = FR ? BT::NFR : 0;
    __builtin_amdgcn_sched_barrier(0);
    if constexpr (N_LDB > 0) loads_b();
    if constexpr (FR) t.template read_frags<BUF, 1>(af1);
    if constexpr (HN) store_next();
    mfma_step_split<BT::TM, BT::TN, FIRST>(acc, af0, bcur[0]);
    sched_interleave<G, N_LDB, NFR, HN ? N_ST : 0>();
    __builtin_amdgcn_sched_barrier(0);

    if constexpr (!(ABL & 4)) __syncthreads();
    if constexpr (N_LDA > 0) loads_a();
    if constexpr (HN && FR) t.template read_frags<BUF ^ 1, 0>(af0);
    mfma_step_split<BT::TM, BT::TN>(acc, af1, bcur[1]);
    sched_interleave<G, N_LDA, HN ? NFR : 0, 0>();
    __builtin_amdgcn_sched_barrier(0);
}

template <int BM_, int BN_, int WM_, int WN_>
struct SplitTileKx : SplitTile<BM_, BN_, WM_, WN_> {
    using Base = SplitTile<BM_, BN_, WM_, WN_>;
    using Base::BM; using Base::TM; using Base::A_LD; using Base::ROWB; using Base::JSTEP; using Base::NT;
    static constexpr int ZROW = BM + 2;
    static constexpr int A_STAGE = (BM + 3) * ROWB;
    static constexpr int LDS_BYTES = 2 * A_STAGE;
    static constexpr int A_LDX = A_LD + 1;
    static_assert(NT / 8 >= 2, "two halo rows");

    int sta_off, sth_off;

    __device__ __forceinline__ explicit SplitTileKx(float* smem) : Base(smem) {
        sta_off = (this->a_r + 1) * ROWB + this->a_q * 8;
        sth_off = (this->a_r == 0 ? 0 : (this->a_r == 1 ? BM + 1 : ZROW)) * ROWB + this->a_q * 8;
    }
    template <int BUF> __device__ __forceinline__ void store_stage(const f32x4 (&a)[A_LDX]) const {
#pragma unroll
        for (int j = 0; j < A_LD; ++j) this->put(this->lds + sta_off + (BUF * A_STAGE + j * JSTEP), a[j]);
        this->put(this->lds + sth_off + BUF * A_STAGE, a[A_LD]);
    }
    template <int ABUF, int S> __device__ __forceinline__ void read_frags_kx(const uint32_t (&fa)[TM], f16x8 (&af)[TM][2]) const {
#pragma unroll
        for (int i = 0; i < TM; ++i)
#pragma unroll
            for (int h = 0; h < 2; ++h)
                af[i][h] = *reinterpret_cast<const f16x8*>(this->lds + fa[i] + (ABUF * A_STAGE + S * 32 + h * 64));
    }
};

}
}
```

### bayesian-yolov3_amd/csrc/wino_split.hip

```cpp
#include <hip/hip_runtime.h>
#include <type_traits>
#include "byolo_kernels.h"
#include "byolo_rng.h"
#include "mfma_pipe.h"
#include "epilogue.h"

namespace byk {

using namespace pipe;

#ifndef BYOLO_WS_ABLATE
#define BYOLO_WS_ABLATE 0
#endif
static constexpr int WS_ABL = BYOLO_WS_ABLATE;
#ifndef BYOLO_WS_FOLD_SKIP
#define BYOLO_WS_FOLD_SKIP 1
#endif
static constexpr bool WS_FOLD_SKIP = BYOLO_WS_FOLD_SKIP != 0;
#ifndef BYOLO_WS_RES_AHEAD
#define BYOLO_WS_RES_AHEAD 1
#endif

#ifndef BYOLO_WS_V_KTMAJOR
#define BYOLO_WS_V_KTMAJOR 1
// ... 153 lines not shown
            for (int j = 0; j < 6; ++j) {
                f32x4 d[4];
                const int x = x0 + j;
#pragma unroll
                for (int i = 0; i < 4; ++i) {
                    const int y = y0 + i;
                    const bool ok = (unsigned)y < (unsigned)p.H && (unsigned)x < (unsigned)p.W && (j < 4 || two);
                    f32x4 a4 = lo[(i + 1) >> 1][(j + 1) >> 1];
                    if (ok && part) a4 += *reinterpret_cast<const f32x4*>(part + ((size_t)y * p.W + x) * p.C);
                    d[i] = ok ? finish(a4, gs, i, j) : f32x4{0.f, 0.f, 0.f, 0.f};
                }
                column(u, j, d);
            }
            emit(s, u);
        }
        if (p.src.status && vmax >= 65520.f) { atomicOr(p.src.status, 1u); atomicMin(p.src.status + 1, (unsigned)p.src.layer_idx); }
    }
}

template <int FEED>
static void launch_input_feed(const WinoParams& p, unsigned grid, hipStream_t st, int twp, uint32_t groups, uint32_t img_lo, uint32_t nsl) {
    const FastDiv a = make_fastdiv((uint32_t)twp), b = make_fastdiv((uint32_t)(p.th * twp)), c = make_fastdiv((uint32_t)p.th), d = make_fastdiv(nsl);
    const int drop = !(p.src.flags & EPI_DROPOUT) ? 0 : (p.src.mask_bits ? 2 : 1);
    if constexpr (FEED == 0) hipLaunchKernelGGL((wino_split_input2_kernel<0, 0>), dim3(grid), dim3(256), 0, st, p, a, b, twp, c, groups, img_lo, d, nsl);
    else if (drop == 0) hipLaunchKernelGGL((wino_split_input2_kernel<FEED, 0>), dim3(grid), dim3(256), 0, st, p, a, b, twp, c, groups, img_lo, d, nsl);
    else if (drop == 1) hipLaunchKernelGGL((wino_split_input2_kernel<FEED, 1>), dim3(grid), dim3(256), 0, st, p, a, b, twp, c, groups, img_lo, d, nsl);
    else hipLaunchKernelGGL((wino_split_input2_kernel<FEED, 2>), dim3(grid), dim3(256), 0, st, p, a, b, twp, c, groups, img_lo, d, nsl);
}

hipError_t launch_wino_split_input(const WinoParams& p, hipStream_t st) {
    const int twp = p.feed == 1 ? p.tw : (p.tw + 1) / 2;
    const uint32_t ns = (uint32_t)(p.P / (p.th * p.tw));
    uint32_t groups = ns, img_lo = 0, nsl = 1;
    if (p.feed < 0 || p.feed > 2) return hipErrorInvalidValue;
    if (p.feed) {
        if (!p.src_low || !p.src.scale || !p.src.shift || p.src_T < 1 || ns < 1 || (p.feed == 2 && ((p.H | p.W) & 1))) return hipErrorInvalidValue;
    }
    if (p.feed == 1) {
        img_lo = (uint32_t)p.s0 / (uint32_t)p.src_T;
        nsl = ((uint32_t)p.src_T + BYOLO_WS_FEED_SLICE - 1) / BYOLO_WS_FEED_SLICE;
        groups = (((uint32_t)p.s0 + ns - 1) / (uint32_t)p.src_T - img_lo + 1) * nsl;
    }
    const uint64_t rows = (uint64_t)groups * p.th * twp + (uint64_t)(p.P_pad - p.P);
    const uint64_t total = rows * (uint64_t)(p.C >> 2);
    const unsigned grid = (unsigned)((total + 255) / 256);
    if (p.feed == 0) launch_input_feed<0>(p, grid, st, twp, groups, img_lo, nsl);
    else if (p.feed == 1) launch_input_feed<1>(p, grid, st, twp, groups, img_lo, nsl);
    else launch_input_feed<2>(p, grid, st, twp, groups, img_lo, nsl);
    return hipGetLastError();
}

__host__ __device__ constexpr int wino_cA(int a, int i) { return a == 0 ? (i < 3 ? 1 : 0) : (i == 0 ? 0 : (i == 1 ? 1 : -1)); }

template <int WINO_BN>
__global__ __launch_bounds__(WINO_BN * 2, 2) void wino_split_kernel(const WinoSplitParams p) {
    extern __shared__ __attribute__((aligned(16))) float smem[];
    __shared__ uint32_t s_claim;
    constexpr int WINO_BM = 64;
    using BT = SplitTile<WINO_BM, WINO_BN, 1, WINO_BN / 32>;
    constexpr int TM = BT::TM, A_LD = BT::A_LD;
    static_assert(BT::TN == 1, "one 32-column block per wave");
    const BT bt(smem);

    const uint32_t nwg = gridDim.x, xcd = blockIdx.x & 7u, slot = blockIdx.x >> 3;
    const uint32_t n_units = (uint32_t)p.units, uq = n_units >> 3, ur = n_units & 7u;
    const uint32_t x0 = xcd * uq + (xcd < ur ? xcd : ur), xn = uq + (xcd < ur ? 1u : 0u);
    const uint32_t ustep = (nwg >> 3) + (xcd < (nwg & 7u) ? 1u : 0u);
    if (slot >= xn) return;
    const uint32_t n_tiles = (uint32_t)p.n_tiles;
    auto unit_of = [&](uint32_t k, uint32_t& rt, uint32_t& ct) __attribute__((always_inline)) { const uint32_t u = x0 + k; rt = fdiv(u, p.d_ntiles); ct = u - rt * n_tiles; };
    auto voff_of = [&](uint32_t rt, uint32_t (&v)[A_LD]) __attribute__((always_inline)) {
#pragma unroll
        for (int j = 0; j < A_LD; ++j) {
            const uint32_t row = (uint32_t)bt.a_r + (uint32_t)(BT::NT / 8) * j;
            if constexpr (BYOLO_WS_V_KTMAJOR != 0) v[j] = rt * (uint32_t)WINO_BM * (uint32_t)p.C * 4u + (row * 32u + (uint32_t)bt.a_q * 4u) * 4u;
            else v[j] = ((rt * (uint32_t)WINO_BM + row) * (uint32_t)p.C + (uint32_t)bt.a_q * 4u) * 4u;
        }
    };
    const __amdgpu_buffer_rsrc_t a_rsrc = make_rsrc(p.v, p.v_bytes);
    const __amdgpu_buffer_rsrc_t w_rsrc = make_rsrc(p.w, p.w_bytes);
    const uint32_t KT = (uint32_t)p.KT;
    const uint32_t w_step = (uint32_t)p.N * BK * 4;

    constexpr int NSET = WINO_BN == 256 ? 4 : 2;
    f32x4 a_reg[NSET][A_LD];
    f16x8 bfr[2][2][1][2];
    uint32_t a_voff[A_LD];
    voff_of(0u, a_voff);
    uint32_t a_base, a_soff, a_kt = 0, a_pt = 0, a_xi_base = 0, a_next_base = 0, a_has_next = 0;
    uint32_t w_soff = 0;
    const uint32_t rt_bytes = (uint32_t)WINO_BM * (uint32_t)p.C * 4u;
    { uint32_t rt, ct; unit_of(slot, rt, ct); a_base = rt * rt_bytes; a_soff = a_base; }
    auto load_a = [&](auto set_tag) __attribute__((always_inline)) {
#pragma unroll
        for (int j = 0; j < A_LD; ++j) a_reg[decltype(set_tag)::value][j] = buffer_load_x4(a_rsrc, a_voff[j], a_soff);
        ++a_kt;
        const uint32_t wrap = a_kt == KT ? 1u : 0u;
        a_kt = wrap ? 0u : a_kt;
        a_xi_base += wrap ? p.xi_stride : 0u;
        a_pt += wrap;
        const uint32_t roll = (a_pt == 16u ? 1u : 0u) & a_has_next;
        a_pt = roll ? 0u : a_pt;
        a_xi_base = roll ? 0u : a_xi_base;
        a_base = roll ? a_next_base : a_base;
        a_soff = a_base + a_xi_base + a_kt * (BYOLO_WS_V_KTMAJOR != 0 ? WINO_BM * BK * 4 : BK * 4);
    };
    auto load_b = [&](auto set_tag) __attribute__((always_inline)) { bt.load_b(bfr[decltype(set_tag)::value], w_rsrc, w_soff); w_soff += w_step; };
// ... 87 lines not shown
        int tid_e = (int)threadIdx.x;
        asm volatile("" : "+v"(tid_e));
        const int e_wn = tid_e >> 6, e_li = tid_e & 31, e_lh = (tid_e >> 5) & 1;
        const int nb = (int)(ct * WINO_BN) + e_wn * 32 + 4 * e_lh;
        float vmax = 0.f;
        f32x4 sc4[4], sf4[4];
#pragma unroll
        for (int g = 0; g < 4; ++g) {
            sc4[g] = *reinterpret_cast<const f32x4*>(p.epi.scale + nb + 8 * g);
            sf4[g] = *reinterpret_cast<const f32x4*>(p.epi.shift + nb + 8 * g);
        }
        const bool keep[4] = {true, true, true, true};
        auto row_of = [&](int k, bool& ok) __attribute__((always_inline)) -> size_t {
            const uint32_t t0 = rt * (uint32_t)WINO_BM + (uint32_t)(k >> 2) * 32u + (uint32_t)e_li;
            const uint32_t t = t0 < (uint32_t)p.P ? t0 : (uint32_t)p.P - 1u;
            const uint32_t s = fdiv(t, p.d_tt), r = t - s * tt;
            const uint32_t ty = fdiv(r, p.d_tw), tx = r - ty * (uint32_t)p.tw;
            const uint32_t oy0 = 2 * ty + (uint32_t)((k >> 1) & 1), ox0 = 2 * tx + (uint32_t)(k & 1);
            ok = t0 < (uint32_t)p.P && oy0 < (uint32_t)p.H && ox0 < (uint32_t)p.W;
            const uint32_t oy = oy0 < (uint32_t)p.H ? oy0 : (uint32_t)p.H - 1u, ox = ox0 < (uint32_t)p.W ? ox0 : (uint32_t)p.W - 1u;
            return (size_t)(((uint64_t)(p.s0 + s) * p.H + oy) * p.W + ox) * p.N + nb;
        };
        constexpr int AHEAD = BYOLO_WS_RES_AHEAD;
        f32x4 rr4[AHEAD][4];
        bool okv[AHEAD + 1]; size_t rowv[AHEAD + 1];
#pragma unroll
        for (int a = 0; a < AHEAD; ++a) {
            rowv[a] = row_of(a, okv[a]);
#pragma unroll
            for (int g = 0; g < 4; ++g) rr4[a][g] = *reinterpret_cast<const f32x4*>(p.residual + rowv[a] + 8 * g);
        }
#pragma unroll
        for (int k = 0; k < 4 * TM; ++k) {
            if (k + AHEAD < 4 * TM) rowv[AHEAD] = row_of(k + AHEAD, okv[AHEAD]);
#pragma unroll
            for (int g = 0; g < 4; ++g) {
                f32x4 a4;
#pragma unroll
                for (int q = 0; q < 4; ++q) a4[q] = Y[k & 3][k >> 2][4 * g + q];
                f32x4 v = epi::bn_act4_pk(a4, sc4[g], sf4[g], keep, slope);
                v += epi::split_decode4(rr4[k % AHEAD][g]);
                if (k + AHEAD < 4 * TM) rr4[k % AHEAD][g] = *reinterpret_cast<const f32x4*>(p.residual + rowv[AHEAD] + 8 * g);
                if (okv[0]) {
                    vmax = epi::absmax4(vmax, v);
                    *reinterpret_cast<f32x4*>(p.y + rowv[0] + 8 * g) = epi::split_encode4(v);
                }
            }
#pragma unroll
            for (int a = 0; a < AHEAD; ++a) { okv[a] = okv[a + 1]; rowv[a] = rowv[a + 1]; }
        }
        if (p.epi.status && vmax >= 65520.f) { atomicOr(p.epi.status, 1u); atomicMin(p.epi.status + 1, (unsigned)p.epi.layer_idx); }
    };

    const bool dyn = p.persist == 2;
    for (uint32_t k = slot, k_next; k < xn; k = k_next) {
        uint32_t rt, ct; unit_of(k, rt, ct);
        k_next = k + ustep;
        if (dyn) { if (threadIdx.x == 0) s_claim = ustep + atomicAdd(p.claims + xcd, 1u); a_has_next = 0; }
        else {
            a_has_next = k_next < xn ? 1u : 0u;
            uint32_t rt2, ct2; unit_of(a_has_next ? k_next : k, rt2, ct2); a_next_base = rt2 * rt_bytes;
        }
        __builtin_amdgcn_sched_barrier(0);
        w_soff = ct * (WINO_BN / 32) * SPLIT_WBLOCK;
        load_b(c0{});
        bt.template read_frags<0, 0>(af0);
#pragma unroll
        for (int o = 0; o < 4; ++o)
#pragma unroll
            for (int i = 0; i < TM; ++i)
#pragma unroll
                for (int r = 0; r < 16; ++r) Y[o][i][r] = 0.f;
            for (int xi = 0; xi < 16; ++xi) {
                run_point();
                if (dyn && xi == 0) {
                    k_next = (uint32_t)__builtin_amdgcn_readfirstlane((int)*reinterpret_cast<volatile uint32_t*>(&s_claim));
                    a_has_next = k_next < xn ? 1u : 0u;
                    uint32_t rt2, ct2; unit_of(a_has_next ? k_next : k, rt2, ct2); a_next_base = rt2 * rt_bytes;
                }
                if constexpr (WS_ABL & 2) { if (xi != 15) continue; }
                const int I = xi >> 2, J = xi & 3;
#pragma unroll
                for (int o = 0; o < 4; ++o) {
                    const float c = (float)(wino_cA(o >> 1, I) * wino_cA(o & 1, J));
                    if constexpr (WS_FOLD_SKIP) { if (c == 0.f) continue; }
                    const f32x2 cc = {c, c};
#pragma unroll
                    for (int i = 0; i < TM; ++i)
#pragma unroll
                        for (int r = 0; r < 16; r += 2) {
                            const f32x2 y2 = __builtin_elementwise_fma(cc, f32x2{M[i][0][r], M[i][0][r + 1]}, f32x2{Y[o][i][r], Y[o][i][r + 1]});
                            Y[o][i][r] = y2[0]; Y[o][i][r + 1] = y2[1];
                        }
                }
            }
        if (p.residual) epilogue_res(rt, ct);
        else if (!(p.epi.flags & EPI_DROPOUT)) epilogue(std::integral_constant<int, 0>{}, rt, ct);
        else if (p.epi.mask_bits) epilogue(std::integral_constant<int, 2>{}, rt, ct);
        else epilogue(std::integral_constant<int, 1>{}, rt, ct);
    }
}

bool wino_split_ok(int C, int N) { return C >= 128 && (C % 128) == 0 && N >= 128 && (N % 128) == 0; }

template <int WINO_BN>
static hipError_t launch_wino_split_bn(const WinoSplitParams& p, hipStream_t st) {
    using BT = SplitTile<64, WINO_BN, 1, WINO_BN / 32>;
    auto k = wino_split_kernel<WINO_BN>;
    static std::atomic<uint64_t> attr_done{0};
    if (hipError_t e = set_dynamic_lds_once(reinterpret_cast<const void*>(k), BT::LDS_BYTES, attr_done); e != hipSuccess) return e;
    const int resident = 256 * (WINO_BN == 256 ? 1 : 2);
    const int grid = (p.persist && p.units > resident) ? resident : p.units;
    hipLaunchKernelGGL(k, dim3((unsigned)grid), dim3(WINO_BN * 2), BT::LDS_BYTES, st, p);
    return hipGetLastError();
}
hipError_t launch_wino_split(const WinoSplitParams& p, hipStream_t st) {
    if (p.bm != 64 || (p.residual && (p.epi.flags & EPI_DROPOUT))) return hipErrorInvalidValue;
    return p.bn == 256 ? launch_wino_split_bn<256>(p, st) : launch_wino_split_bn<128>(p, st);
}

}
```

### include/byolo.h

```cpp
#ifndef BYOLO_H_
#define BYOLO_H_

#include <stddef.h>
#include <stdint.h>

#ifdef __cplusplus
extern "C" {
#endif

#define BYOLO_API __attribute__((visibility("default")))

#define BYOLO_OK 0
#define BYOLO_ERR_ARG (-1)
#define BYOLO_ERR_STATE (-2)
#define BYOLO_ERR_HIP (-3)
#define BYOLO_ERR_NOMEM (-4)
#define BYOLO_ERR_RANGE (-5)

typedef struct byolo byolo_t;

enum { BYOLO_DET_STANDARD = 0, BYOLO_DET_ALEATORIC = 1, BYOLO_DET_EPISTEMIC = 2 };
enum { BYOLO_NMS_AGNOSTIC = 0, BYOLO_NMS_TWO_CLASS = 1, BYOLO_NMS_PER_CLASS = 2 };
#define BYOLO_NMS_MAX_CLASSES 128
enum { BYOLO_NORM_BN = 1, BYOLO_NORM_DROPOUT = 2 };

typedef struct byolo_cfg {
    int32_t img_h, img_w, img_c;
    int32_t cls_cnt;
    float   drop_prob;
    int32_t max_out;
    float   iou_thresh;
    int32_t nms_mode;
    int32_t keep_all_outputs;
} byolo_cfg;

BYOLO_API int32_t byolo_create(const byolo_cfg* cfg, int32_t device, byolo_t** out);
BYOLO_API int32_t byolo_destroy(byolo_t* h);
enum { BYOLO_PREC_F32 = 0, BYOLO_PREC_SPLIT_F16 = 1 };
BYOLO_API int32_t byolo_set_precision(byolo_t* h, int32_t precision);
BYOLO_API int32_t byolo_get_precision(const byolo_t* h);
BYOLO_API const char* byolo_precision_note(const byolo_t* h);
BYOLO_API const char* byolo_last_error(const byolo_t* h);
BYOLO_API const char* byolo_version(void);
#define BYOLO_ABI_VERSION 7
BYOLO_API int32_t byolo_abi_version(void);

typedef struct byolo_plan_opts {
    int32_t struct_bytes;
    int32_t graphs;
    int32_t serialize_convs;
    int32_t serialize_heads;
    int32_t dedup;
    int32_t lowmain;
    int32_t kx3, p1;
    int32_t b2b;
    int32_t kx3_wide;
    int32_t wino_split;
    int32_t wino_split_min_c;
    int32_t wino_split_bn;
    int32_t wino_split_rounds;
    int32_t winograd;
    int32_t wino_fused;
    int32_t stream1x1;
    int32_t gemm_stream;
    int32_t ksplit;
    int32_t streamk;
    int32_t plain_epilogue;
    int32_t wshift_per_layer;
    int32_t nms_general;
    int32_t wino_split_persist;
    int32_t wino_split_feed;
    float   wino_split_min_gflop;
    float   wino_split_chunk_mb;
    float   wino_min_gflop;
    float   wino_chunk_mb;
    float   wino_min_ratio;
} byolo_plan_opts;
BYOLO_API int32_t byolo_get_plan_opts(const byolo_t* h, byolo_plan_opts* out);
BYOLO_API int32_t byolo_set_plan_opts(byolo_t* h, const byolo_plan_opts* opts);
BYOLO_API int32_t byolo_graph_stats(const byolo_t* h, int32_t* n_graphs, int64_t* replays, int64_t* captures, int64_t* updates);


BYOLO_API int32_t byolo_add_conv(byolo_t* h, const char* scope, int32_t filters, int32_t ksize, int32_t stride,
                       int32_t norm_flags);
BYOLO_API int32_t byolo_add_residual(byolo_t* h, int32_t shortcut);
BYOLO_API int32_t byolo_add_route(byolo_t* h, const int32_t* routes, int32_t n_routes);
BYOLO_API int32_t byolo_add_upsample(byolo_t* h);
BYOLO_API int32_t byolo_add_stack(byolo_t* h, int32_t src);
BYOLO_API int32_t byolo_add_detection(byolo_t* h, const char* scope, int32_t kind, const float* priors_hw );

BYOLO_API int32_t byolo_mark_backbone_end(byolo_t* h);

BYOLO_API int32_t byolo_num_params(const byolo_t* h);
BYOLO_API int32_t byolo_param_info(const byolo_t* h, int32_t i, const char** name, int32_t* ndim, int64_t shape[4]);
BYOLO_API int32_t byolo_set_param(byolo_t* h, const char* name, const float* h_data, int64_t count);
BYOLO_API int32_t byolo_get_param(const byolo_t* h, const char* name, float* h_data, int64_t count);
BYOLO_API int32_t byolo_finalize(byolo_t* h);

BYOLO_API int32_t byolo_num_layers(const byolo_t* h);
BYOLO_API int32_t byolo_num_boxes(const byolo_t* h, int64_t* n_boxes, int32_t* row_len);
BYOLO_API int32_t byolo_workspace_bytes(byolo_t* h, int32_t B, int32_t T, size_t* out);
BYOLO_API int32_t byolo_plan_num(byolo_t* h, int32_t B, int32_t T, int32_t inject, int32_t* n_steps, int32_t* n_tensors, int64_t* arena_bytes);
BYOLO_API int32_t byolo_plan_step(byolo_t* h, int32_t step, int32_t* out_tensor, int32_t* fuses_next, int32_t reads[8], int32_t* n_reads);
BYOLO_API int32_t byolo_plan_tensor(byolo_t* h, int32_t tensor, int64_t* offset, int64_t* bytes, int32_t* read_after_the_steps);
BYOLO_API int32_t byolo_forward(byolo_t* h, const float* d_img, int32_t B, int32_t T, uint64_t seed, int32_t dropout_on,
                      const uint32_t* d_mask_bits, void* d_workspace, size_t workspace_bytes,
                      float* d_boxes, float* d_rows, int32_t* d_kept, int32_t* d_count, void* stream);
BYOLO_API int32_t byolo_num_dropout(const byolo_t* h);
BYOLO_API int32_t byolo_mask_layout(byolo_t* h, int32_t B, int32_t T, int32_t ordinal, int64_t* bit_offset, int64_t* elements);
BYOLO_API int32_t byolo_set_async(byolo_t* h, int32_t on);
BYOLO_API int32_t byolo_status(byolo_t* h, void* stream, uint32_t* flags, int32_t* layer);
BYOLO_API int32_t byolo_clear_status(byolo_t* h, void* stream);
BYOLO_API int32_t byolo_set_first_image(byolo_t* h, int64_t first_image);
BYOLO_API int32_t byolo_set_tshard(byolo_t* h, int32_t t0, int32_t T_total);
BYOLO_API int32_t byolo_finish_tshard(byolo_t* h, float* d_sums, int32_t B, int32_t T_total, void* stream);
BYOLO_API int32_t byolo_max_images(byolo_t* h, int32_t T, int32_t* max_images);
BYOLO_API int32_t byolo_layer_output(const byolo_t* h, int32_t idx, const float** d_ptr, int64_t shape[4]);
BYOLO_API int32_t byolo_copy_layer_output(const byolo_t* h, int32_t idx, float* d_dst, int64_t count, void* stream);

BYOLO_API int32_t byolo_decode(byolo_t* h, int32_t kind, const float* d_raw, int32_t B, int32_t T, int32_t lh, int32_t lw,
                     const float* priors_hw , int32_t layer_id, float* d_boxes,
                     int64_t n_total, int64_t box_base, void* stream);
BYOLO_API int32_t byolo_epistemic_stats(byolo_t* h, const float* d_raw, int32_t B, int32_t T, int32_t lh, int32_t lw,
                                        float* d_ev_loc, float* d_epi_covar, float* d_obj_samples, float* d_cls_samples,
// ... 245 lines not shown
```

Baseline: 388.4.

## Fuse detection-head 1x1 conv into preceding split Winograd 3x3 kernel via partial slabs

When a split-f16 Winograd 3x3 conv whose output is read only by a 1x1 detection conv is found, the Winograd kernel applies BN/leaky/dropout in registers, stages the activation in LDS, and runs the head's 1x1 GEMM per 256-channel slab, writing fp32 partial sums. A small slab-reduce kernel then sums the slabs and applies the head epilogue. This is meant to avoid writing and rereading the large 3x3 activation tensor and a separate head GEMM launch. The cost is extra slab workspace, a non-persistent larger-LDS kernel variant, and added planning complexity for calibration and workspace sizing.

Measured after the change: 391.8 (median of 6 runs). About the same (+0.9%).

```diff
diff --git a/bayesian-yolov3_amd/byolo/_lib.py b/bayesian-yolov3_amd/byolo/_lib.py
--- a/bayesian-yolov3_amd/byolo/_lib.py
+++ b/bayesian-yolov3_amd/byolo/_lib.py
@@ -29,7 +29,7 @@
     _fields_ = [(n, ctypes.c_int32) for n in (
         "struct_bytes", "graphs", "serialize_convs", "serialize_heads", "dedup", "lowmain", "kx3", "p1", "b2b", "kx3_wide", "wino_split", "wino_split_min_c",
         "wino_split_bn", "wino_split_rounds", "winograd", "wino_fused", "stream1x1", "gemm_stream", "ksplit", "streamk",
-        "plain_epilogue", "wshift_per_layer", "nms_general", "wino_split_persist", "wino_split_feed")] + [(n, ctypes.c_float) for n in (
+        "plain_epilogue", "wshift_per_layer", "nms_general", "wino_split_persist", "wino_split_feed", "wino_follow")] + [(n, ctypes.c_float) for n in (
         "wino_split_min_gflop", "wino_split_chunk_mb", "wino_min_gflop", "wino_chunk_mb", "wino_min_ratio")]
 
 
diff --git a/bayesian-yolov3_amd/csrc/byolo_api.hip b/bayesian-yolov3_amd/csrc/byolo_api.hip
--- a/bayesian-yolov3_amd/csrc/byolo_api.hip
+++ b/bayesian-yolov3_amd/csrc/byolo_api.hip
@@ -46,7 +46,7 @@
     o.struct_bytes = (int32_t)sizeof o;
     o.graphs = 1; o.serialize_convs = 1; o.serialize_heads = 1; o.dedup = 1; o.lowmain = 1; o.kx3 = 1; o.p1 = 1; o.b2b = 1; o.kx3_wide = 0;
     o.wino_split = 1; o.wino_split_min_c = 256; o.wino_split_bn = 0; o.wino_split_rounds = 0;
-    o.winograd = 1; o.wino_fused = 1; o.stream1x1 = 1; o.gemm_stream = 1; o.ksplit = -1; o.streamk = 1; o.plain_epilogue = 1; o.wino_split_persist = 0; o.wino_split_feed = 3;
+    o.winograd = 1; o.wino_fused = 1; o.stream1x1 = 1; o.gemm_stream = 1; o.ksplit = -1; o.streamk = 1; o.plain_epilogue = 1; o.wino_split_persist = 0; o.wino_split_feed = 3; o.wino_follow = 1;
     o.wino_split_min_gflop = 30.f; o.wino_split_chunk_mb = 1500.f; o.wino_min_gflop = 10.f; o.wino_chunk_mb = 800.f; o.wino_min_ratio = 80.f;
 }
 static void plan_opts_from_env(byolo_plan_opts& o) {
@@ -58,7 +58,7 @@
     geti("BYOLO_WINO_SPLIT", o.wino_split); geti("BYOLO_WINO_SPLIT_MIN_C", o.wino_split_min_c); geti("BYOLO_WINO_SPLIT_BN", o.wino_split_bn);
     geti("BYOLO_WINO_SPLIT_ROUNDS", o.wino_split_rounds); geti("BYOLO_WINOGRAD", o.winograd);
     geti("BYOLO_WINO_FUSED", o.wino_fused); geti("BYOLO_STREAM1X1", o.stream1x1); geti("BYOLO_GEMM_STREAM", o.gemm_stream);
-    geti("BYOLO_KSPLIT", o.ksplit); geti("BYOLO_STREAMK", o.streamk); geti("BYOLO_PLAIN_EPILOGUE", o.plain_epilogue); geti("BYOLO_WINO_SPLIT_PERSIST", o.wino_split_persist); geti("BYOLO_WINO_SPLIT_FEED", o.wino_split_feed);
+    geti("BYOLO_KSPLIT", o.ksplit); geti("BYOLO_STREAMK", o.streamk); geti("BYOLO_PLAIN_EPILOGUE", o.plain_epilogue); geti("BYOLO_WINO_SPLIT_PERSIST", o.wino_split_persist); geti("BYOLO_WINO_SPLIT_FEED", o.wino_split_feed); geti("BYOLO_WINO_FOLLOW", o.wino_follow);
     geti("BYOLO_WSHIFT_PER_LAYER", o.wshift_per_layer); geti("BYOLO_NMS_GENERAL", o.nms_general);
     getf("BYOLO_WINO_SPLIT_MIN_GFLOP", o.wino_split_min_gflop); getf("BYOLO_WINO_SPLIT_CHUNK_MB", o.wino_split_chunk_mb);
     getf("BYOLO_WINO_MIN_GFLOP", o.wino_min_gflop); getf("BYOLO_WINO_CHUNK_MB", o.wino_chunk_mb); getf("BYOLO_WINO_MIN_RATIO", o.wino_min_ratio);
@@ -85,7 +85,7 @@
     if (o->graphs < 0 || o->graphs > 2 || o->serialize_convs < 0 || o->serialize_convs > 2 || o->b2b < 0 || o->b2b > 2 || o->kx3_wide < 0 || o->kx3_wide > 2 ||
         o->wino_split < 0 || o->wino_split > 2 || o->winograd < 0 || o->winograd > 2 || o->wino_fused < 0 || o->wino_fused > 2 || o->stream1x1 < 0 || o->stream1x1 > 2 ||
         o->streamk < 0 || o->streamk > 2 || o->ksplit < -1 || o->ksplit > 64 || (o->wino_split_bn != 0 && o->wino_split_bn != 128 && o->wino_split_bn != 256) ||
-        o->wino_split_rounds < 0 || o->wino_split_persist < 0 || o->wino_split_persist > 2 || o->wino_split_feed < 0 || o->wino_split_feed > 3 || !(o->wino_split_chunk_mb > 0.f) || !(o->wino_chunk_mb > 0.f) || !(o->wino_split_min_gflop >= 0.f) || !(o->wino_min_gflop >= 0.f) || !(o->wino_min_ratio >= 0.f))
+        o->wino_split_rounds < 0 || o->wino_split_persist < 0 || o->wino_split_persist > 2 || o->wino_split_feed < 0 || o->wino_split_feed > 3 || o->wino_follow < 0 || o->wino_follow > 1 || !(o->wino_split_chunk_mb > 0.f) || !(o->wino_chunk_mb > 0.f) || !(o->wino_split_min_gflop >= 0.f) || !(o->wino_min_gflop >= 0.f) || !(o->wino_min_ratio >= 0.f))
         return fail(h, BYOLO_ERR_ARG, "byolo_set_plan_opts: a field outside its range (include/byolo.h)");
     const byolo_plan_opts& c = h->opts;
     const bool repack = (o->wshift_per_layer != 0) != (c.wshift_per_layer != 0) || (o->dedup != 0) != (c.dedup != 0) || (o->lowmain != 0) != (c.lowmain != 0) || (o->kx3 != 0) != (c.kx3 != 0) || (o->p1 != 0) != (c.p1 != 0);
@@ -499,6 +499,16 @@
         st.wino_ok = !l.direct && l.op == OP_CONV && l.ksize == 3 && l.stride == 1 && st.mode == STEP_NORMAL &&
                      st.in.n == 1 && st.in.s[0].sh == 0 && !st.in.s[0].tile && (l.Cin % 32) == 0 && (N % 4) == 0;
     }
+    { const std::vector<int> readers = count_readers(h);
+      for (int si = 0; si < (int)h->steps.size(); ++si) {
+          const int ri = follow_reader(h, si, readers);
+          if (ri < 0) continue;
+          const Layer& l = h->layers[h->steps[si].layer];
+          h->aux.push_back({l.H, l.W, l.filters / 256 * layer_pitch(h->layers[h->steps[ri].layer]), l.stacked});
+          h->steps[si].slab_tensor = n + (int)h->aux.size() - 1;
+          h->last_use.push_back(-1);
+      }
+    }
     h->maxC = 1;
     for (const auto& l : h->layers) h->maxC = std::max(h->maxC, l.C);
     decide_loops(h);
@@ -699,7 +709,7 @@
 }
 
 static int32_t run_wino_split(byolo_t* h, const Step& s, const Layer& l, const ConvParams& c, const WinoPlan& wp, double algo_flops,
-                              char* ws, hipStream_t st, const WinoParams* feed = nullptr) {
+                              char* ws, hipStream_t st, const WinoParams* feed = nullptr, const ConvParams* head = nullptr, float* slabs = nullptr) {
     const bool prof = h->profiling >= 2;
     int32_t rc;
     const int S = c.M / (l.H * l.W), tt = wp.th * wp.tw;
@@ -729,6 +739,11 @@
         const int chunk_idx = s0 / wp.chunk;
         f.persist = (h->opts.wino_split_persist == 2 && c.counters && chunk_idx < CNT_PER_STEP / 8) ? 2 : (h->opts.wino_split_persist ? 1 : 0);
         f.claims = c.counters ? c.counters + 8 * chunk_idx : nullptr;
+        if (head) {
+            f.f_w = head->wpk; f.f_w_bytes = head->w_bytes; f.f_Npad = head->Npad; f.f_ld = head->ldc;
+            f.slabs = slabs; f.slab_stride = (uint64_t)c.M * head->ldc;
+            f.y = nullptr; f.persist = 0; f.claims = nullptr;
+        }
         f.d_ntiles = make_fastdiv((uint32_t)f.n_tiles); f.d_tt = w.d_tt; f.d_tw = w.d_tw;
         if (prof && (rc = mark_launch(h, s.layer, 140, (int64_t)rows, c.N, c.C0, algo_flops * ns / S, st, 1, wp.bn))) return rc;
         HIPCHK(h, launch_wino_split(f, st));
@@ -1168,11 +1183,28 @@
             ++si;
             continue;
         }
+        if (h->plan.follow_src[si] >= 0) {
+            const Step& ps = h->steps[h->plan.follow_src[si]];
+            const int n_slabs = h->layers[ps.layer].filters / 256;
+            const float* slabs = reinterpret_cast<const float*>(ws + h->plan.off[ps.slab_tensor]);
+            if (per_step) { rc = mark_launch(h, s.layer, -6, p.M, l.filters, p.C0, algo, st, n_slabs, 0); if (rc) return rc; }
+            HIPCHK(h, launch_slab_reduce(slabs, (uint64_t)p.M * p.ldc, n_slabs, p.M, p.ldc, p.epi.scale, p.epi.shift, p.dst, st));
+            continue;
+        }
         if (h->plan.wino[si].chunk > 0 && h->precision == 1) {
             WinoParams fw;
             const bool fed = h->plan.feed_src[si] >= 0;
             if (fed) { rc = feed_params((size_t)h->plan.feed_src[si], fw); if (rc) return rc; }
-            rc = run_wino_split(h, s, l, p, h->plan.wino[si], algo, ws, st, fed ? &fw : nullptr); if (rc) return rc;
+            ConvParams hd; int htile = 0; double halgo = 0.0;
+            const bool fol = h->plan.follow[si] != 0;
+            if (fol) {
+                size_t ri = si + 1;
+                while (ri < h->steps.size() && h->plan.follow_src[ri] != (int)si) ++ri;
+                if (ri >= h->steps.size()) return fail(h, BYOLO_ERR_STATE, "byolo_forward: a follow pair without its second step");
+                rc = prep(ri, hd, htile, halgo); if (rc) return rc;
+            }
+            rc = run_wino_split(h, s, l, p, h->plan.wino[si], algo, ws, st, fed ? &fw : nullptr, fol ? &hd : nullptr,
+                                fol ? reinterpret_cast<float*>(ws + h->plan.off[s.slab_tensor]) : nullptr); if (rc) return rc;
             continue;
         }
         if (h->plan.wino[si].chunk > 0) { rc = run_winograd(h, s, l, p, h->plan.wino[si], tile, algo, ws, st); if (rc) return rc; continue; }
@@ -1494,7 +1526,9 @@
                                       void* stream) {
     int32_t rc = check_run(h, B, 1, "byolo_calibrate_bn"); if (rc) return rc;
     if (!d_img || !d_workspace) return fail(h, BYOLO_ERR_ARG, "byolo_calibrate_bn: null argument");
+    h->plan.B = -1; h->plan.no_follow = true;
     make_plan(h, B, 1);
+    h->plan.no_follow = false;
     if (workspace_bytes < h->plan.total) return fail(h, BYOLO_ERR_NOMEM, "byolo_calibrate_bn: workspace %zu < %zu", workspace_bytes, h->plan.total);
     for (size_t si = 0; si < h->steps.size(); ++si) {
         const Step& s = h->steps[si];
@@ -1584,6 +1618,7 @@
         if (h) {
             bool doctored = rc != BYOLO_OK;
             for (char f : h->plan.feed) doctored = doctored || f != 0;
+            doctored = doctored || h->plan.follow_held;
             if (doctored) h->plan.B = -1;
         }
         return rc;
diff --git a/bayesian-yolov3_amd/csrc/byolo_internal.h b/bayesian-yolov3_amd/csrc/byolo_internal.h
--- a/bayesian-yolov3_amd/csrc/byolo_internal.h
+++ b/bayesian-yolov3_amd/csrc/byolo_internal.h
@@ -74,6 +74,7 @@
     bool low = false;
     int low_tensor = -1;
     int raw_tensor = -1;
+    int slab_tensor = -1;
     size_t w_off = 0; int Npad = 0, tile = 0;
     bool wino_ok = false;
     size_t wino_off = 0;
@@ -99,6 +100,9 @@
     std::vector<char> fuse;
     std::vector<char> feed;
     std::vector<int> feed_src;
+    std::vector<char> follow;
+    std::vector<int> follow_src;
+    bool no_follow = false, follow_held = false;
     size_t wino_off = 0;
 };
 static constexpr int CNT_PER_STEP = 1024;
@@ -219,6 +223,8 @@
 int64_t tensor_bytes(const byolo_t* h, int id, int B, int T);
 void step_geometry(const byolo_t* h, const Step& st, int B, int T, int* M, int* KT);
 void decide_loops(byolo_t* h);
+std::vector<int> count_readers(const byolo_t* h);
+int follow_reader(const byolo_t* h, int si, const std::vector<int>& readers);
 void make_plan(byolo_t* h, int B, int T, bool inject = false);
 int64_t piece_cap(const byolo_t* h, int32_t T);
 int32_t check_run(byolo_t* h, int32_t B, int32_t T, const char* what, bool need_device = true);
diff --git a/bayesian-yolov3_amd/csrc/byolo_kernels.h b/bayesian-yolov3_amd/csrc/byolo_kernels.h
--- a/bayesian-yolov3_amd/csrc/byolo_kernels.h
+++ b/bayesian-yolov3_amd/csrc/byolo_kernels.h
@@ -109,8 +109,13 @@
     unsigned* claims;
     int units;
     FastDiv d_ntiles, d_tt, d_tw;
+    const float* f_w; uint32_t f_w_bytes;
+    float* slabs;
+    uint64_t slab_stride;
+    int f_Npad, f_ld;
 };
 bool wino_split_ok(int C, int N);
+hipError_t launch_slab_reduce(const float* slabs, uint64_t slab_stride, int n_slabs, int64_t M, int ld, const float* scale, const float* shift, float* out, hipStream_t st);
 hipError_t launch_wino_split_input(const WinoParams& p, hipStream_t st);
 hipError_t launch_wino_split(const WinoSplitParams& p, hipStream_t st);
 struct GemmStreamParams {
diff --git a/bayesian-yolov3_amd/csrc/byolo_plan.hip b/bayesian-yolov3_amd/csrc/byolo_plan.hip
--- a/bayesian-yolov3_amd/csrc/byolo_plan.hip
+++ b/bayesian-yolov3_amd/csrc/byolo_plan.hip
@@ -32,6 +32,33 @@
                  (st.mode == STEP_NORMAL || st.mode == STEP_REP);
         st.p1 = p1_on && l.ksize == 1 && l.stride == 1 && st.in.n == 1 && st.in.s[0].layer >= 0 && st.Npad >= 64;
     }
+}
+
+std::vector<int> count_readers(const byolo_t* h) {
+    std::vector<int> readers(h->layers.size() + h->aux.size(), 0);
+    for (const Step& s : h->steps) {
+        for (int k = 0; k < s.in.n; ++k) if (s.in.s[k].layer >= 0) ++readers[s.in.s[k].layer];
+        if (s.addend_tensor >= 0) ++readers[s.addend_tensor];
+        if (s.low_tensor >= 0) ++readers[s.low_tensor];
+        const Layer& l = h->layers[s.layer];
+        if (s.is_conv() && l.fused_residual >= 0) ++readers[h->layers[l.fused_residual].ref[0]];
+    }
+    return readers;
+}
+
+int follow_reader(const byolo_t* h, int si, const std::vector<int>& readers) {
+    const Step& s = h->steps[si];
+    const Layer& l = h->layers[s.layer];
+    if (!s.wino_ok || s.mode != STEP_NORMAL || l.op != OP_CONV || (l.filters % 256) || s.Npad != l.filters || l.fused_residual >= 0 || !wino_split_ok(s.c_hi - s.c_lo, l.filters)) return -1;
+    const int t = s.out_tensor, ri = t < (int)h->layers.size() ? h->last_use[t] : -1;
+    if (ri <= si || readers[t] != 1) return -1;
+    const Step& r = h->steps[ri];
+    const Layer& l2 = h->layers[r.layer];
+    const bool ok = r.is_conv() && r.mode == STEP_NORMAL && l2.op == OP_DETECTION && !l2.direct && l2.ksize == 1 && l2.stride == 1 && r.in.n == 1 &&
+                    r.in.s[0].layer == t && !r.in.s[0].tile && r.in.s[0].sh == 0 && r.in.s[0].C == l.filters && r.c_lo == 0 && r.c_hi == l.filters &&
+                    l2.fused_residual < 0 && l2.drop_ordinal < 0 && r.Npad <= 64 && (layer_pitch(l2) % 4) == 0 && layer_pitch(l2) <= r.Npad &&
+                    l2.H == l.H && l2.W == l.W && l2.stacked == l.stacked;
+    return ok ? ri : -1;
 }
 
 void make_plan(byolo_t* h, int B, int T, bool inject) {
@@ -141,15 +168,8 @@
     }
     p.feed.assign(h->steps.size(), 0); p.feed_src.assign(h->steps.size(), -1);
     std::vector<int> last_use = h->last_use;
+    const std::vector<int> readers = count_readers(h);
     if (h->precision == 1 && h->opts.wino_split_feed && !h->cfg.keep_all_outputs) {
-        std::vector<int> readers(n, 0);
-        for (const Step& s : h->steps) {
-            for (int k = 0; k < s.in.n; ++k) if (s.in.s[k].layer >= 0) ++readers[s.in.s[k].layer];
-            if (s.addend_tensor >= 0) ++readers[s.addend_tensor];
-            if (s.low_tensor >= 0) ++readers[s.low_tensor];
-            const Layer& l = h->layers[s.layer];
-            if (s.is_conv() && l.fused_residual >= 0) ++readers[h->layers[l.fused_residual].ref[0]];
-        }
         for (int si = 0; si < (int)h->steps.size(); ++si) {
             const Step& s = h->steps[si];
             const int kind = s.mode == STEP_REP ? 1 : s.mode == STEP_FINISH ? 2 : 0;
@@ -164,9 +184,21 @@
             else { last_use[s.low_tensor] = ri; if (s.addend_tensor >= 0) last_use[s.addend_tensor] = ri; }
         }
     }
+    p.follow.assign(h->steps.size(), 0); p.follow_src.assign(h->steps.size(), -1); p.follow_held = false;
+    if (h->precision == 1 && h->opts.wino_follow && !inject && !h->cfg.keep_all_outputs) {
+        for (int si = 0; si < (int)h->steps.size(); ++si) {
+            const Step& s = h->steps[si];
+            if (s.slab_tensor < 0 || p.wino[si].chunk <= 0 || p.wino[si].bn != 256 || p.fuse[si] || p.feed[si]) continue;
+            const int ri = follow_reader(h, si, readers);
+            if (ri < 0 || p.feed[ri] || p.fuse[ri] || (ri > 0 && p.fuse[ri - 1])) continue;
+            if (p.no_follow) { p.follow_held = true; continue; }
+            p.follow[si] = 1; p.follow_src[ri] = si;
+            last_use[s.slab_tensor] = ri;
+        }
+    }
     for (int si = 0; si < (int)h->steps.size(); ++si) {
         const Layer& l = h->layers[h->steps[si].layer];
-        const int t = p.feed[si] == 1 ? h->steps[si].raw_tensor : h->steps[si].out_tensor;
+        const int t = p.feed[si] == 1 ? h->steps[si].raw_tensor : p.follow[si] ? h->steps[si].slab_tensor : h->steps[si].out_tensor;
         if (!(si > 0 && p.fuse[si - 1]) && p.feed[si] != 2) p.off[t] = alloc(tensor_bytes(h, t, B, T));
         if (p.fuse[si]) { const int t2 = h->steps[si + 1].out_tensor; p.off[t2] = alloc(tensor_bytes(h, t2, B, T)); }
         if (h->cfg.keep_all_outputs) continue;
@@ -334,6 +366,12 @@
         h->plan.B = -1;
         make_plan(h, B, T, true);
         h->wsm_total = h->plan.total; h->wsm_B = B; h->wsm_T = T; h->wsm_epoch = h->plan_epoch;
+        if (keep.follow_src.size() && std::any_of(keep.follow.begin(), keep.follow.end(), [](char f) { return f != 0; })) {
+            h->plan.B = -1; h->plan.no_follow = true;
+            make_plan(h, B, T, false);
+            h->plan.no_follow = false;
+            h->wsm_total = std::max(h->wsm_total, h->plan.total);
+        }
         h->plan = keep; h->plan_inject = false;
     }
     *out = std::max(h->plan.total, h->wsm_total);
@@ -366,12 +404,15 @@
         const Step& ps = h->steps[fs];
         if (h->plan.feed[fs] == 1) reads[n++] = ps.raw_tensor;
         else { reads[n++] = ps.low_tensor; if (ps.addend_tensor >= 0) reads[n++] = ps.addend_tensor; }
+    } else if (step < (int32_t)h->plan.follow_src.size() && h->plan.follow_src[step] >= 0) {
+        reads[n++] = h->steps[h->plan.follow_src[step]].slab_tensor;
     } else
     for (int k = 0; k < st.in.n; ++k) if (st.in.s[k].layer >= 0) reads[n++] = st.in.s[k].layer;
     if (st.addend_tensor >= 0) reads[n++] = st.addend_tensor;
     if (st.low_tensor >= 0) reads[n++] = st.low_tensor;
     if (st.is_conv() && st.mode != STEP_PARTIAL && l.fused_residual >= 0) reads[n++] = h->layers[l.fused_residual].ref[0];
-    if (out_tensor) *out_tensor = fk == 1 ? st.raw_tensor : fk == 2 ? st.low_tensor : st.out_tensor;
+    const bool fol = step < (int32_t)h->plan.follow.size() && h->plan.follow[step];
+    if (out_tensor) *out_tensor = fk == 1 ? st.raw_tensor : fk == 2 ? st.low_tensor : fol ? st.slab_tensor : st.out_tensor;
     if (fuses_next) *fuses_next = (step < (int32_t)h->plan.fuse.size() && h->plan.fuse[step]) ? 1 : 0;
     if (n_reads) *n_reads = n;
     return BYOLO_OK;
diff --git a/bayesian-yolov3_amd/csrc/conv_igemm.hip b/bayesian-yolov3_amd/csrc/conv_igemm.hip
--- a/bayesian-yolov3_amd/csrc/conv_igemm.hip
+++ b/bayesian-yolov3_amd/csrc/conv_igemm.hip
@@ -549,25 +549,7 @@
         for (int r = 0; r < 16; ++r) acc2[i][0][r] = 0.f;
     const __amdgpu_buffer_rsrc_t w_rsrc = make_rsrc(p.f_wpk, p.f_w_bytes);
     const uint32_t w_step = (uint32_t)p.f_Npad * BK * 4;
-    f16x8 bfr[2][2][1][2];
-    f16x8 afr[2][TM2][2];
-    bt.load_b(bfr[0], w_rsrc, 0u);
-    bt.template read_frags<0, 0>(afr[0]);
-    auto step2 = [&](auto s_tag) {
-        constexpr int S = decltype(s_tag)::value, KT2 = S >> 1, H = S & 1;
-        __builtin_amdgcn_sched_barrier(0);
-        if constexpr (H == 0 && KT2 < 7) bt.load_b(bfr[(KT2 + 1) & 1], w_rsrc, (uint32_t)(KT2 + 1) * w_step);
-        if constexpr (S < 15) bt.template read_frags<((S + 1) >> 1) & 7, (S + 1) & 1>(afr[(S + 1) & 1]);
-        __builtin_amdgcn_sched_barrier(0);
-        mfma_step_split<TM2, 1>(acc2, afr[S & 1], bfr[KT2 & 1][H]);
-        __builtin_amdgcn_sched_barrier(0);
-    };
-    step2(std::integral_constant<int, 0>{}); step2(std::integral_constant<int, 1>{}); step2(std::integral_constant<int, 2>{});
-    step2(std::integral_constant<int, 3>{}); step2(std::integral_constant<int, 4>{}); step2(std::integral_constant<int, 5>{});
-    step2(std::integral_constant<int, 6>{}); step2(std::integral_constant<int, 7>{}); step2(std::integral_constant<int, 8>{});
-    step2(std::integral_constant<int, 9>{}); step2(std::integral_constant<int, 10>{}); step2(std::integral_constant<int, 11>{});
-    step2(std::integral_constant<int, 12>{}); step2(std::integral_constant<int, 13>{}); step2(std::integral_constant<int, 14>{});
-    step2(std::integral_constant<int, 15>{});
+    follower_gemm(bt, acc2, w_rsrc, 0u, w_step);
     __syncthreads();
     auto follower = [&](auto drop_tag, auto split_tag) {
         constexpr bool DROP = decltype(drop_tag)::value, SPLIT_OUT = decltype(split_tag)::value;
diff --git a/bayesian-yolov3_amd/csrc/conv_kernels.hip b/bayesian-yolov3_amd/csrc/conv_kernels.hip
--- a/bayesian-yolov3_amd/csrc/conv_kernels.hip
+++ b/bayesian-yolov3_amd/csrc/conv_kernels.hip
@@ -412,4 +412,42 @@
     return hipGetLastError();
 }
 
-}
+template <int NS>
+__global__ __launch_bounds__(256) void slab_reduce_kernel(const f32x4* __restrict__ slabs, const uint64_t stride4, const int n_slabs, const int64_t total4,
+                                                          const uint32_t ld4, const FastDiv d_ld4, const float* __restrict__ scale, const float* __restrict__ shift,
+                                                          f32x4* __restrict__ out) {
+    const int64_t i = (int64_t)blockIdx.x * 256 + threadIdx.x;
+    if (i >= total4) return;
+    const uint32_t c4 = (uint32_t)i - fdiv((uint32_t)i, d_ld4) * ld4;
+    f32x4 s;
+    if constexpr (NS > 0) {
+        f32x4 v[NS];
+#pragma unroll
+        for (int j = 0; j < NS; ++j) v[j] = __builtin_nontemporal_load(slabs + (size_t)j * stride4 + i);
+        s = v[0];
+#pragma unroll
+        for (int j = 1; j < NS; ++j) s += v[j];
+    } else {
+        s = slabs[i];
+        for (int j = 1; j < n_slabs; ++j) s += slabs[(size_t)j * stride4 + i];
+    }
+    const f32x4 sc = *reinterpret_cast<const f32x4*>(scale + 4 * c4), sf = *reinterpret_cast<const f32x4*>(shift + 4 * c4);
+    f32x4 v;
+#pragma unroll
+    for (int q = 0; q < 4; ++q) v[q] = __builtin_fmaf(s[q], sc[q], sf[q]);
+    out[i] = v;
+}
+hipError_t launch_slab_reduce(const float* slabs, uint64_t slab_stride, int n_slabs, int64_t M, int ld, const float* scale, const float* shift, float* out, hipStream_t st) {
+    const int64_t total4 = M * (ld / 4);
+    if (n_slabs < 1 || ld < 4 || (ld & 3) || (slab_stride & 3) || M < 1 || total4 >= ((int64_t)1 << 31)) return hipErrorInvalidValue;
+    const dim3 grid((unsigned)((total4 + 255) / 256));
+    const FastDiv d = make_fastdiv((uint32_t)(ld / 4));
+    const f32x4* s4 = reinterpret_cast<const f32x4*>(slabs);
+    f32x4* o4 = reinterpret_cast<f32x4*>(out);
+    if (n_slabs == 2) hipLaunchKernelGGL(slab_reduce_kernel<2>, grid, dim3(256), 0, st, s4, slab_stride / 4, n_slabs, total4, (uint32_t)(ld / 4), d, scale, shift, o4);
+    else if (n_slabs == 4) hipLaunchKernelGGL(slab_reduce_kernel<4>, grid, dim3(256), 0, st, s4, slab_stride / 4, n_slabs, total4, (uint32_t)(ld / 4), d, scale, shift, o4);
+    else hipLaunchKernelGGL(slab_reduce_kernel<0>, grid, dim3(256), 0, st, s4, slab_stride / 4, n_slabs, total4, (uint32_t)(ld / 4), d, scale, shift, o4);
+    return hipGetLastError();
+}
+
+}
diff --git a/bayesian-yolov3_amd/csrc/mfma_pipe.h b/bayesian-yolov3_amd/csrc/mfma_pipe.h
--- a/bayesian-yolov3_amd/csrc/mfma_pipe.h
+++ b/bayesian-yolov3_amd/csrc/mfma_pipe.h
@@ -1,6 +1,7 @@
 #pragma once
 #include <hip/hip_runtime.h>
 #include <stdint.h>
+#include <type_traits>
 #include "byolo_kernels.h"
 
 namespace byk {
@@ -230,6 +231,31 @@
     __builtin_amdgcn_sched_barrier(0);
 }
 
+template <class BT2>
+__device__ __forceinline__ void follower_gemm(const BT2& bt, f32x16 (&acc2)[BT2::TM][1], const __amdgpu_buffer_rsrc_t w_rsrc, const uint32_t w_base, const uint32_t w_step) {
+    constexpr int TM2 = BT2::TM;
+    static_assert(BT2::TN == 1, "one column block per wave");
+    f16x8 bfr[2][2][1][2];
+    f16x8 afr[2][TM2][2];
+    bt.load_b(bfr[0], w_rsrc, w_base);
+    bt.template read_frags<0, 0>(afr[0]);
+    auto step2 = [&](auto s_tag) {
+        constexpr int S = decltype(s_tag)::value, KT2 = S >> 1, H = S & 1;
+        __builtin_amdgcn_sched_barrier(0);
+        if constexpr (H == 0 && KT2 < 7) bt.load_b(bfr[(KT2 + 1) & 1], w_rsrc, w_base + (uint32_t)(KT2 + 1) * w_step);
+        if constexpr (S < 15) bt.template read_frags<((S + 1) >> 1) & 7, (S + 1) & 1>(afr[(S + 1) & 1]);
+        __builtin_amdgcn_sched_barrier(0);
+        mfma_step_split<TM2, 1>(acc2, afr[S & 1], bfr[KT2 & 1][H]);
+        __builtin_amdgcn_sched_barrier(0);
+    };
+    step2(std::integral_constant<int, 0>{}); step2(std::integral_constant<int, 1>{}); step2(std::integral_constant<int, 2>{});
+    step2(std::integral_constant<int, 3>{}); step2(std::integral_constant<int, 4>{}); step2(std::integral_constant<int, 5>{});
+    step2(std::integral_constant<int, 6>{}); step2(std::integral_constant<int, 7>{}); step2(std::integral_constant<int, 8>{});
+    step2(std::integral_constant<int, 9>{}); step2(std::integral_constant<int, 10>{}); step2(std::integral_constant<int, 11>{});
+    step2(std::integral_constant<int, 12>{}); step2(std::integral_constant<int, 13>{}); step2(std::integral_constant<int, 14>{});
+    step2(std::integral_constant<int, 15>{});
+}
+
 template <int BM_, int BN_, int WM_, int WN_>
 struct SplitTileKx : SplitTile<BM_, BN_, WM_, WN_> {
     using Base = SplitTile<BM_, BN_, WM_, WN_>;
diff --git a/bayesian-yolov3_amd/csrc/wino_split.hip b/bayesian-yolov3_amd/csrc/wino_split.hip
--- a/bayesian-yolov3_amd/csrc/wino_split.hip
+++ b/bayesian-yolov3_amd/csrc/wino_split.hip
@@ -229,7 +229,7 @@
 
 __host__ __device__ constexpr int wino_cA(int a, int i) { return a == 0 ? (i < 3 ? 1 : 0) : (i == 0 ? 0 : (i == 1 ? 1 : -1)); }
 
-template <int WINO_BN>
+template <int WINO_BN, int FOLLOW = 0>
 __global__ __launch_bounds__(WINO_BN * 2, 2) void wino_split_kernel(const WinoSplitParams p) {
     extern __shared__ __attribute__((aligned(16))) float smem[];
     __shared__ uint32_t s_claim;
@@ -423,6 +423,81 @@
         if (p.epi.status && vmax >= 65520.f) { atomicOr(p.epi.status, 1u); atomicMin(p.epi.status + 1, (unsigned)p.epi.layer_idx); }
     };
 
+    auto follow_pass = [&](auto h_tag, uint32_t rt, uint32_t ct) __attribute__((always_inline)) {
+        constexpr int HP = decltype(h_tag)::value;
+        constexpr int ROWB = BT::ROWB, IMG_BUF = 128 * ROWB;
+        using BT2 = SplitTile<128, 64, 4, 2>;
+        static_assert(FOLLOW == 0 || (WINO_BN == 256 && TM == 2), "the 8-wave workgroup: 64 tiles x 256 channels");
+        const float slope = (p.epi.flags & EPI_LEAKY) ? 0.1f : 1.f;
+        const uint32_t tt = (uint32_t)(p.th * p.tw);
+        int tid_e = (int)threadIdx.x;
+        asm volatile("" : "+v"(tid_e));
+        const int e_wn = tid_e >> 6, e_li = tid_e & 31, e_lh = (tid_e >> 5) & 1;
+        char* lds = reinterpret_cast<char*>(smem);
+        auto pix_of = [&](const uint32_t t0, const uint32_t o, bool& ok) __attribute__((always_inline)) -> uint64_t {
+            const uint32_t t = t0 < (uint32_t)p.P ? t0 : (uint32_t)p.P - 1u;
+            const uint32_t s = fdiv(t, p.d_tt), r = t - s * tt;
+            const uint32_t ty = fdiv(r, p.d_tw), tx = r - ty * (uint32_t)p.tw;
+            const uint32_t oy = 2 * ty + (o >> 1), ox = 2 * tx + (o & 1u);
+            ok = t0 < (uint32_t)p.P && oy < (uint32_t)p.H && ox < (uint32_t)p.W;
+            return ((uint64_t)(p.s0 + s) * p.H + oy) * p.W + ox;
+        };
+        {
+            const int nb = (int)(ct * WINO_BN) + e_wn * 32 + 4 * e_lh;
+            float vmax = 0.f;
+            f32x4 sc4[4], sf4[4];
+#pragma unroll
+            for (int g = 0; g < 4; ++g) {
+                sc4[g] = *reinterpret_cast<const f32x4*>(p.epi.scale + nb + 8 * g);
+                sf4[g] = *reinterpret_cast<const f32x4*>(p.epi.shift + nb + 8 * g);
+            }
+#pragma unroll
+            for (int i = 0; i < TM; ++i)
+#pragma unroll
+                for (int ol = 0; ol < 2; ++ol) {
+                    constexpr int O0 = 2 * HP;
+                    bool ok;
+                    const uint64_t pix = pix_of(rt * (uint32_t)WINO_BM + (uint32_t)i * 32u + (uint32_t)e_li, (uint32_t)(O0 + ol), ok);
+                    const epi::DropRow drow(p.epi.idx_base + pix * (uint64_t)p.N + (uint64_t)nb, p.epi.k1);
+                    char* row = lds + e_wn * IMG_BUF + (ol * 64 + i * 32 + e_li) * ROWB + e_lh * 8;
+#pragma unroll
+                    for (int g = 0; g < 4; ++g) {
+                        f32x4 a4;
+#pragma unroll
+                        for (int q = 0; q < 4; ++q) a4[q] = Y[O0 + ol][i][4 * g + q];
+                        bool keep[4] = {true, true, true, true};
+                        if constexpr (FOLLOW == 2) epi::keep4(drow, 8 * g, p.epi.k0, p.epi.thr, keep);
+                        const f32x4 v = epi::bn_act4_pk(a4, sc4[g], sf4[g], keep, slope);
+                        const float vm = epi::absmax4(vmax, v);
+                        vmax = ok ? vm : vmax;
+                        const f32x4 e = epi::split_encode4(v);
+                        *reinterpret_cast<f32x2*>(row + 16 * g) = f32x2{e[0], e[1]};
+                        *reinterpret_cast<f32x2*>(row + 16 * g + 64) = f32x2{e[2], e[3]};
+                    }
+                }
+            if (p.epi.status && vmax >= 65520.f) { atomicOr(p.epi.status, 1u); atomicMin(p.epi.status + 1, (unsigned)p.epi.layer_idx); }
+        }
+        __syncthreads();
+        const BT2 bt2(smem, tid_e);
+        f32x16 acc2[1][1];
+#pragma unroll
+        for (int r = 0; r < 16; ++r) acc2[0][0][r] = 0.f;
+        const uint32_t f_step = (uint32_t)p.f_Npad * BK * 4;
+        follower_gemm(bt2, acc2, make_rsrc(p.f_w, p.f_w_bytes), ct * 8u * f_step, f_step);
+        if constexpr (HP == 0) __syncthreads();
+        {
+            bool ok;
+            const uint64_t pix = pix_of(rt * (uint32_t)WINO_BM + (uint32_t)(bt2.wm & 1) * 32u + (uint32_t)bt2.li, (uint32_t)(2 * HP + (bt2.wm >> 1)), ok);
+            const int n0 = bt2.wn * 32 + 4 * bt2.lh;
+            float* d = p.slabs + (size_t)ct * p.slab_stride + (size_t)pix * p.f_ld + n0;
+            if (ok) {
+#pragma unroll
+                for (int g = 0; g < 4; ++g)
+                    if (n0 + 8 * g < p.f_ld) *reinterpret_cast<f32x4*>(d + 8 * g) = f32x4{acc2[0][0][4 * g], acc2[0][0][4 * g + 1], acc2[0][0][4 * g + 2], acc2[0][0][4 * g + 3]};
+            }
+        }
+    };
+
     const bool dyn = p.persist == 2;
     for (uint32_t k = slot, k_next; k < xn; k = k_next) {
         uint32_t rt, ct; unit_of(k, rt, ct);
@@ -465,7 +540,8 @@
                         }
                 }
             }
-        if (p.residual) epilogue_res(rt, ct);
+        if constexpr (FOLLOW != 0) { follow_pass(c0{}, rt, ct); follow_pass(c1{}, rt, ct); }
+        else if (p.residual) epilogue_res(rt, ct);
         else if (!(p.epi.flags & EPI_DROPOUT)) epilogue(std::integral_constant<int, 0>{}, rt, ct);
         else if (p.epi.mask_bits) epilogue(std::integral_constant<int, 2>{}, rt, ct);
         else epilogue(std::integral_constant<int, 1>{}, rt, ct);
@@ -485,8 +561,23 @@
     hipLaunchKernelGGL(k, dim3((unsigned)grid), dim3(WINO_BN * 2), BT::LDS_BYTES, st, p);
     return hipGetLastError();
 }
+template <int FOLLOW>
+static hipError_t launch_wino_split_follow(const WinoSplitParams& p, hipStream_t st) {
+    constexpr int LDS_BYTES = 8 * 128 * LD * 4;
+    static_assert(LDS_BYTES >= SplitTile<64, 256, 1, 8>::LDS_BYTES, "the image covers the V stages");
+    auto k = wino_split_kernel<256, FOLLOW>;
+    static std::atomic<uint64_t> attr_done{0};
+    if (hipError_t e = set_dynamic_lds_once(reinterpret_cast<const void*>(k), LDS_BYTES, attr_done); e != hipSuccess) return e;
+    hipLaunchKernelGGL(k, dim3((unsigned)p.units), dim3(512), LDS_BYTES, st, p);
+    return hipGetLastError();
+}
 hipError_t launch_wino_split(const WinoSplitParams& p, hipStream_t st) {
     if (p.bm != 64 || (p.residual && (p.epi.flags & EPI_DROPOUT))) return hipErrorInvalidValue;
+    if (p.f_w) {
+        if (p.bn != 256 || p.residual || p.epi.mask_bits || p.persist || !p.slabs || p.f_ld < 4 || (p.f_ld & 3) || p.f_ld > 64 || p.f_Npad < 32 || (p.f_Npad & 31) ||
+            (uint64_t)p.f_w_bytes < (uint64_t)p.N / 32 * p.f_Npad * BK * 4) return hipErrorInvalidValue;
+        return (p.epi.flags & EPI_DROPOUT) ? launch_wino_split_follow<2>(p, st) : launch_wino_split_follow<1>(p, st);
+    }
     return p.bn == 256 ? launch_wino_split_bn<256>(p, st) : launch_wino_split_bn<128>(p, st);
 }
 
diff --git a/include/byolo.h b/include/byolo.h
--- a/include/byolo.h
+++ b/include/byolo.h
@@ -70,6 +70,7 @@
     int32_t nms_general;
     int32_t wino_split_persist;
     int32_t wino_split_feed;
+    int32_t wino_follow;
     float   wino_split_min_gflop;
     float   wino_split_chunk_mb;
     float   wino_min_gflop;
```
